# uber-research/UPSNet

Hardware: NVIDIA H100
Metric: panoptic images/sec at 1024x2048 (higher is better)
Workload: dtype bf16x3

## Files before the change

upsnet_b200/csrc/dcn_win.cu:

```cuda
#include <cuda.h>
#include <cuda_bf16.h>

#include "common.cuh"
#include "tc_ptx.cuh"
#include "tc_params.cuh"

namespace ups {

constexpr int DW_BM = 128;
constexpr int DW_WW = 32, DW_WH = 20;
constexpr int DW_PLANE = DW_WW * DW_WH * 32;
constexpr int DW_WIN_BYTES = 2 * DW_PLANE;
constexpr int DW_WIN_BUFS = 2;
constexpr int DW_KHW = 9;
constexpr int DW_GROUPS = 2;
constexpr int DW_EPI_PITCH = 36;
constexpr uint32_t DW_EPI_BYTES = DW_BM * DW_EPI_PITCH * 4;

constexpr uint32_t DW_OFF_BARS = 0;
constexpr uint32_t DW_OFF_STATS = 192;
constexpr uint32_t DW_OFF_ORG = 256;
constexpr uint32_t DW_OFF_TW = 512;
constexpr uint32_t DW_OFF_TP = DW_OFF_TW + DW_KHW * DW_BM * 16;
constexpr uint32_t DW_OFF_STAGES = DW_OFF_TP + DW_KHW * DW_BM * 4;
static_assert(DW_OFF_STAGES % 1024 == 0, "stage buffers need 1024-byte alignment (SWIZZLE_128B)");

template <int BN> struct DwCfg {
  static constexpr int NCW = BN == 128 ? 2 : 1;
  static constexpr int FRAGS = 2 / NCW;
  static constexpr int BK = BN == 128 ? 32 : 64;
  static constexpr int SPK = BK / 16;
  static constexpr int ROWB = BK * 2;
  static constexpr int CONSUMERS = 128 * NCW;
  static constexpr int WARP_TMAB = CONSUMERS / 32, WARP_TMAW = WARP_TMAB + 1, WARP_PROD0 = WARP_TMAB + 4;
  static constexpr int GROUP = 4 * (SPK / 2) * 32;
  static constexpr int PRODUCERS = GROUP * DW_GROUPS;
  static constexpr int THREADS = WARP_PROD0 * 32 + PRODUCERS;
  static constexpr int WARPGROUPS = THREADS / 128;
  static constexpr int REGS_LAUNCH = 16384 / (32 * ((THREADS / 32 + 3) / 4)) / 8 * 8;
  static constexpr int REGS_TMA = 32, REGS_CONSUMER = 128;
  static_assert(NCW * REGS_CONSUMER + REGS_TMA + (PRODUCERS / 128) * REGS_LAUNCH <= WARPGROUPS * REGS_LAUNCH,
                "setmaxnreg budgets exceed the CTA's register allocation");
  static constexpr int TABLE_IT = (DW_KHW * DW_BM + PRODUCERS - 1) / PRODUCERS;
  static constexpr uint32_t A_BYTES = 2 * DW_BM * ROWB;
  static constexpr uint32_t B_BYTES = BN * ROWB;
  static constexpr uint32_t STAGE_BYTES = 2 * B_BYTES + A_BYTES;
  static_assert(STAGE_BYTES % 1024 == 0, "stages must keep the 1024-byte alignment of the swizzled tiles");
  static constexpr int STAGES = BN == 128 ? 3 : 2;
  static_assert(STAGES <= 3, "the barrier map holds three stages");
  static constexpr uint32_t OFF_WIN = DW_OFF_STAGES + STAGES * STAGE_BYTES;
  static constexpr uint32_t OFF_EPI = OFF_WIN + DW_WIN_BUFS * DW_WIN_BYTES;
  static constexpr uint32_t SMEM = OFF_EPI + DW_EPI_BYTES + 1024;
  static_assert(SMEM <= 227 * 1024, "shared memory exceeds 227 KB");
};
template <int ROWB> __device__ __forceinline__ uint32_t dw_chunk(uint32_t j, uint32_t r) {
  return ROWB == 128 ? (j ^ (r & 7u)) : (j ^ ((r >> 1) & 3u));
}

struct DwParams {
  const void* x;
  const float* offset;
  const float* mask;
  const float* bias;
  void* y;
  int N, H, W, Cin, Cout, Cout_pad, Ho, Wo, ph, pw, dh, dw, relu, BN, tile_w, tile_h;
};

template <int BN>
__global__ void __launch_bounds__(DwCfg<BN>::THREADS, 1)
dcn_win_kernel(const __grid_constant__ CUtensorMap tm_x, const __grid_constant__ CUtensorMap tm_w, const __grid_constant__ DwParams p) {
  using C = DwCfg<BN>;
  constexpr int DW_PRODUCERS = C::PRODUCERS, DW_CONSUMERS = C::CONSUMERS;
  constexpr int DW_WARP_TMAB = C::WARP_TMAB, DW_WARP_TMAW = C::WARP_TMAW, DW_WARP_PROD0 = C::WARP_PROD0;
  constexpr int DW_BK = C::BK, SPK = C::SPK, ROWB = C::ROWB;
  extern __shared__ __align__(1024) uint8_t smem_dyn[];
  const uint32_t raw = smem_u32(smem_dyn);
  const uint32_t base = (raw + 1023u) & ~1023u;
  uint8_t* sm = smem_dyn + (base - raw);

  const int tid = threadIdx.x, warp = tid >> 5, lane = tid & 31;
  const uint32_t b_bytes = C::B_BYTES;
  const uint32_t stage_bytes = C::STAGE_BYTES;
  constexpr uint32_t NST = C::STAGES, NWB = DW_WIN_BUFS;
  const uint32_t win_base = base + C::OFF_WIN;
  float* stf = reinterpret_cast<float*>(sm + C::OFF_EPI);
  const uint32_t bar_fa = base + DW_OFF_BARS;
  const uint32_t bar_fb = bar_fa + 24;
  const uint32_t bar_em = bar_fa + 48;
  const uint32_t bar_wf = bar_fa + 104;
  const uint32_t bar_we = bar_fa + 120;
  const uint32_t bar_og = bar_fa + 136;
  int* stats = reinterpret_cast<int*>(sm + DW_OFF_STATS);
  int4* org = reinterpret_cast<int4*>(sm + DW_OFF_ORG);
  float4* tw = reinterpret_cast<float4*>(sm + DW_OFF_TW);
  int* tp = reinterpret_cast<int*>(sm + DW_OFF_TP);

  const int HoWo = p.Ho * p.Wo;
  const int nsc = p.Cin / 16;
  const int num_kb = nsc * DW_KHW / SPK;
  const int n_tiles = p.Cout_pad / BN;
  const int TW = p.tile_w, TH = p.tile_h;
  const int tw_shift = TW == 16 ? 4 : 3;
  const int tiles_w = (p.Wo + TW - 1) / TW, tiles_h = (p.Ho + TH - 1) / TH;
  const long long num_tiles = (long long)p.N * tiles_w * tiles_h * n_tiles;

  if (warp == 0) {
    if (lane == 0) {
      for (int s = 0; s < C::STAGES; ++s) {
        mbar_init(bar_fa + 8 * s, C::GROUP / 32);
        mbar_init(bar_fb + 8 * s, 1);
        mbar_init(bar_em + 8 * s, DW_CONSUMERS / 32);
      }
      for (int s = 0; s < 2; ++s) {
        mbar_init(bar_wf + 8 * s, 1);
        mbar_init(bar_we + 8 * s, DW_PRODUCERS / 32);
        mbar_init(bar_og + 8 * s, 1);
      }
      fence_mbar_init();
      for (int i = 0; i < 2; ++i) {
        stats[i * 8 + 0] = 0x7fffffff; stats[i * 8 + 1] = 0x7fffffff;
        stats[i * 8 + 2] = -0x7fffffff; stats[i * 8 + 3] = -0x7fffffff;
        stats[i * 8 + 4] = 0; stats[i * 8 + 5] = 0; stats[i * 8 + 6] = 0; stats[i * 8 + 7] = 0;
      }
    }
    __syncwarp();
  }
  if (warp == DW_WARP_TMAB && lane == 0) prefetch_tmap(&tm_w);
  if (warp == DW_WARP_TMAW && lane == 0) prefetch_tmap(&tm_x);
  __syncthreads();

  if (warp >= DW_WARP_PROD0) {
    const int pt = tid - DW_WARP_PROD0 * 32;
    const int pw = warp - DW_WARP_PROD0;
    const int group = pw / (C::GROUP / 32);
    const int u = (pw >> 2) & (SPK / 2 - 1);
    const int quad = pw & 3;
    const int r = quad * 32 + lane;
    const __nv_bfloat16* xh = reinterpret_cast<const __nv_bfloat16*>(p.x);
    uint32_t g0 = 0, wf0 = 0;
    uint32_t wf_ready = 0;
    uint32_t tile_it = 0;
    for (long long tile = blockIdx.x; tile < num_tiles; tile += gridDim.x, ++tile_it) {
      const long long mt = tile / n_tiles;
      const int tx = (int)(mt % tiles_w), ty = (int)((mt / tiles_w) % tiles_h), n = (int)(mt / ((long long)tiles_w * tiles_h));
      const int par = (int)(tile_it & 1u);
      constexpr int TIT = C::TABLE_IT;
      float4 ewv[TIT];
      int ehl[TIT], ewl[TIT];
      bool evalid[TIT];
      int mnw = 0x7fffffff, mnh = 0x7fffffff, mxw = -0x7fffffff, mxh = -0x7fffffff, sw_ = 0, sh_ = 0, cnt = 0;
#pragma unroll
      for (int it = 0; it < TIT; ++it) {
        const int e = pt + it * DW_PRODUCERS;
        ewv[it] = make_float4(0.f, 0.f, 0.f, 0.f);
        ehl[it] = 0; ewl[it] = 0; evalid[it] = false;
        if (e < DW_KHW * DW_BM) {
          const int tap = e >> 7, rr = e & 127;
          const int ry = rr >> tw_shift;
          const int wo = tx * TW + (rr & (TW - 1)), ho = ty * TH + ry;
          if (ry < TH && wo < p.Wo && ho < p.Ho) {
            const int pp = ho * p.Wo + wo;
            const int ki = tap / 3, kj = tap - ki * 3;
            const float* offp = p.offset + ((size_t)n * 2 * DW_KHW + 2 * tap) * HoWo + pp;
            const float oh = __ldg(offp), ow = __ldg(offp + HoWo);
            const float h = (float)(ho - p.ph + ki * p.dh) + oh;
            const float w = (float)(wo - p.pw + kj * p.dw) + ow;
            if (h > -1.f && w > -1.f && h < (float)p.H && w < (float)p.W) {
              const int hl = (int)floorf(h), wl = (int)floorf(w), hh = hl + 1, wh = wl + 1;
              const float lh = h - hl, lw = w - wl, ch = 1.f - lh, cw = 1.f - lw;
              const bool t_ok = hl >= 0, b_ok = hh <= p.H - 1, l_ok = wl >= 0, r_ok = wh <= p.W - 1;
              float m = 1.f;
              if (p.mask) m = __ldg(p.mask + ((size_t)n * DW_KHW + tap) * HoWo + pp);
              ewv[it].x = (t_ok && l_ok) ? ch * cw * m : 0.f;
              ewv[it].y = (t_ok && r_ok) ? ch * lw * m : 0.f;
              ewv[it].z = (b_ok && l_ok) ? lh * cw * m : 0.f;
              ewv[it].w = (b_ok && r_ok) ? lh * lw * m : 0.f;
              ehl[it] = hl; ewl[it] = wl; evalid[it] = true;
              mnw = min(mnw, wl); mxw = max(mxw, wl + 1); mnh = min(mnh, hl); mxh = max(mxh, hl + 1);
              sw_ += wl; sh_ += hl; ++cnt;
            }
          }
        }
      }
      mnw = __reduce_min_sync(0xffffffffu, mnw); mnh = __reduce_min_sync(0xffffffffu, mnh);
      mxw = __reduce_max_sync(0xffffffffu, mxw); mxh = __reduce_max_sync(0xffffffffu, mxh);
      sw_ = __reduce_add_sync(0xffffffffu, sw_); sh_ = __reduce_add_sync(0xffffffffu, sh_);
      cnt = __reduce_add_sync(0xffffffffu, cnt);
      if (lane == 0 && cnt > 0) {
        int* st = stats + par * 8;
        atomicMin(st + 0, mnw); atomicMin(st + 1, mnh); atomicMax(st + 2, mxw); atomicMax(st + 3, mxh);
        atomicAdd(st + 4, sw_); atomicAdd(st + 5, sh_); atomicAdd(st + 6, cnt);
      }
      named_bar<1, DW_PRODUCERS>();
      int ox = 0, oy = 0;
      {
        const int* st = stats + par * 8;
        const int c = st[6];
        if (c > 0) {
          const int a = st[0], b = st[1], cc = st[2], d = st[3];
          ox = (cc - a + 1 <= DW_WW) ? a : (int)floorf((float)st[4] / (float)c + 1.0f) - DW_WW / 2;
          oy = (d - b + 1 <= DW_WH) ? b : (int)floorf((float)st[5] / (float)c + 1.0f) - DW_WH / 2;
        }
      }
#pragma unroll
      for (int it = 0; it < TIT; ++it) {
        const int e = pt + it * DW_PRODUCERS;
        if (e < DW_KHW * DW_BM) {
          int code = 0;
          if (evalid[it]) {
            const int dx = ewl[it] - ox, dy = ehl[it] - oy;
            if (dx >= 0 && dx + 1 < DW_WW && dy >= 0 && dy + 1 < DW_WH) code = (dy * DW_WW + dx) * 32;
            else code = (int)(0x80000000u | ((uint32_t)(ehl[it] + 1) << 15) | (uint32_t)(ewl[it] + 1));
          }
          tw[e] = ewv[it];
          tp[e] = code;
        }
      }
      if (pt == 0) {
        org[par] = make_int4(ox, oy, n, 0);
        int* so = stats + (par ^ 1) * 8;
        so[0] = 0x7fffffff; so[1] = 0x7fffffff; so[2] = -0x7fffffff; so[3] = -0x7fffffff; so[4] = 0; so[5] = 0; so[6] = 0;
        mbar_arrive(bar_og + 8 * par);
      }
      named_bar<1, DW_PRODUCERS>();
      const __nv_bfloat16* ximg = xh + (size_t)n * p.H * p.W * (size_t)(2 * p.Cin);

      int rel = 0;
      for (int kb = (int)((uint32_t)(group - (int)g0) & 1u); kb < num_kb; kb += DW_GROUPS) {
        const uint32_t g = g0 + (uint32_t)kb;
        const uint32_t s = g % NST, it = g / NST;
        mbar_wait(bar_em + 8 * s, (it & 1u) ^ 1u);
        const uint32_t a_row = base + DW_OFF_STAGES + s * stage_bytes + 2 * b_bytes + (uint32_t)r * (uint32_t)ROWB;
#pragma unroll 1
        for (int pass = 0; pass < 4; ++pass) {
          const int sl = 2 * u + (pass >> 1), half = pass & 1;
          const int q = kb * SPK + sl;
          const int sc = q / DW_KHW, tap = q - sc * DW_KHW;
          const uint32_t wf = wf0 + (uint32_t)sc;
          if (wf >= wf_ready) {
            mbar_wait(bar_wf + 8 * (wf % NWB), (wf / NWB) & 1u);
            wf_ready = wf + 1;
          }
          const uint32_t wbuf = win_base + (wf % NWB) * (uint32_t)DW_WIN_BYTES;
          const int code = tp[tap * DW_BM + r];
          const uint32_t a_off = dw_chunk<ROWB>((uint32_t)(sl * 2 + half), (uint32_t)r) << 4;
          const float4 wv = tw[tap * DW_BM + r];
          uint4 hc[4], lc[4];
          if (code >= 0) {
            const uint32_t cl = (uint32_t)code, cr = cl + 32u;
            const uint32_t al = wbuf + cl + ((((cl >> 7) & 1u) ^ (uint32_t)half) << 4);
            const uint32_t ar = wbuf + cr + ((((cr >> 7) & 1u) ^ (uint32_t)half) << 4);
            hc[0] = lds128(al); hc[1] = lds128(ar); hc[2] = lds128(al + DW_WW * 32); hc[3] = lds128(ar + DW_WW * 32);
            lc[0] = lds128(al + DW_PLANE); lc[1] = lds128(ar + DW_PLANE);
            lc[2] = lds128(al + DW_PLANE + DW_WW * 32); lc[3] = lds128(ar + DW_PLANE + DW_WW * 32);
          } else {
            const int hl = (int)(((uint32_t)code >> 15) & 0xffffu) - 1, wl = (int)((uint32_t)code & 0x7fffu) - 1;
            const int h0 = max(hl, 0), h1 = min(hl + 1, p.H - 1), w0 = max(wl, 0), w1 = min(wl + 1, p.W - 1);
            const size_t pc = (size_t)(2 * p.Cin);
            const int cg = sc * 16 + half * 8;
            const __nv_bfloat16* b00 = ximg + ((size_t)h0 * p.W + w0) * pc + cg;
            const __nv_bfloat16* b01 = ximg + ((size_t)h0 * p.W + w1) * pc + cg;
            const __nv_bfloat16* b10 = ximg + ((size_t)h1 * p.W + w0) * pc + cg;
            const __nv_bfloat16* b11 = ximg + ((size_t)h1 * p.W + w1) * pc + cg;
            hc[0] = __ldg(reinterpret_cast<const uint4*>(b00)); lc[0] = __ldg(reinterpret_cast<const uint4*>(b00 + p.Cin));
            hc[1] = __ldg(reinterpret_cast<const uint4*>(b01)); lc[1] = __ldg(reinterpret_cast<const uint4*>(b01 + p.Cin));
            hc[2] = __ldg(reinterpret_cast<const uint4*>(b10)); lc[2] = __ldg(reinterpret_cast<const uint4*>(b10 + p.Cin));
            hc[3] = __ldg(reinterpret_cast<const uint4*>(b11)); lc[3] = __ldg(reinterpret_cast<const uint4*>(b11 + p.Cin));
          }
          const float wf4[4] = {wv.x, wv.y, wv.z, wv.w};
          unsigned long long acc[4] = {0ull, 0ull, 0ull, 0ull};
          __nv_bfloat162 lacc[4];
#pragma unroll
          for (int i = 0; i < 4; ++i) {
            const uint32_t hw_[4] = {hc[i].x, hc[i].y, hc[i].z, hc[i].w};
            const uint32_t lw_[4] = {lc[i].x, lc[i].y, lc[i].z, lc[i].w};
            const __nv_bfloat162 wb = __float2bfloat162_rn(wf4[i]);
            unsigned long long wp;
            asm("mov.b64 %0, {%1, %1};" : "=l"(wp) : "r"(__float_as_uint(wf4[i])));
#pragma unroll
            for (int qq = 0; qq < 4; ++qq) {
              unsigned long long hp;
              asm("mov.b64 %0, {%1, %2};" : "=l"(hp) : "r"(hw_[qq] << 16), "r"(hw_[qq] & 0xffff0000u));
              acc[qq] = f32x2_fma(wp, hp, acc[qq]);
              const __nv_bfloat162 lv = *reinterpret_cast<const __nv_bfloat162*>(&lw_[qq]);
              lacc[qq] = i == 0 ? __hmul2(wb, lv) : __hfma2(wb, lv, lacc[qq]);
            }
          }
          uint32_t ohi[4], olo[4];
#pragma unroll
          for (int qq = 0; qq < 4; ++qq) {
            const uint32_t lw = *reinterpret_cast<const uint32_t*>(&lacc[qq]);
            unsigned long long lp;
            asm("mov.b64 %0, {%1, %2};" : "=l"(lp) : "r"(lw << 16), "r"(lw & 0xffff0000u));
            acc[qq] = f32x2_add(acc[qq], lp);
            uint32_t a0, a1;
            asm("mov.b64 {%0, %1}, %2;" : "=r"(a0), "=r"(a1) : "l"(acc[qq]));
            const float v0 = __uint_as_float(a0), v1 = __uint_as_float(a1);
            ohi[qq] = pack_bf16x2(v0, v1);
            olo[qq] = pack_bf16x2(v0 - __uint_as_float(ohi[qq] << 16), v1 - __uint_as_float(ohi[qq] & 0xffff0000u));
          }
          sts128(a_row + a_off, make_uint4(ohi[0], ohi[1], ohi[2], ohi[3]));
          sts128(a_row + DW_BM * ROWB + a_off, make_uint4(olo[0], olo[1], olo[2], olo[3]));
        }
        fence_proxy_async();
        __syncwarp();
        if (lane == 0) {
          mbar_arrive(bar_fa + 8 * s);
          while (rel < nsc && DW_KHW * (rel + 1) <= SPK * (kb + DW_GROUPS)) {
            mbar_arrive(bar_we + 8 * ((wf0 + (uint32_t)rel) % NWB));
            ++rel;
          }
        }
        rel = __shfl_sync(0xffffffffu, rel, 0);
      }
      if (lane == 0) {
        while (rel < nsc) { mbar_arrive(bar_we + 8 * ((wf0 + (uint32_t)rel) % NWB)); ++rel; }
      }
      __syncwarp();
      g0 += (uint32_t)num_kb;
      wf0 += (uint32_t)nsc;
    }
  } else if (warp >= DW_WARP_TMAB) {
    setmaxnreg_dec<C::REGS_TMA>();
    if (warp == DW_WARP_TMAW && lane == 0) {
      uint32_t wf = 0, ti = 0;
      for (long long tile = blockIdx.x; tile < num_tiles; tile += gridDim.x, ++ti) {
        const uint32_t par = ti & 1u;
        mbar_wait(bar_og + 8 * par, (ti >> 1) & 1u);
        const volatile int* ov = reinterpret_cast<const volatile int*>(&org[par]);
        const int4 o = make_int4(ov[0], ov[1], ov[2], 0);
        for (int f = 0; f < nsc; ++f, ++wf) {
          const uint32_t b = wf % NWB;
          mbar_wait(bar_we + 8 * b, ((wf / NWB) & 1u) ^ 1u);
          mbar_arrive_expect_tx(bar_wf + 8 * b, (uint32_t)DW_WIN_BYTES);
          const uint32_t dst = win_base + b * (uint32_t)DW_WIN_BYTES;
          tma_load_4d(dst, &tm_x, bar_wf + 8 * b, f * 16, o.x, o.y, o.z);
          tma_load_4d(dst + (uint32_t)DW_PLANE, &tm_x, bar_wf + 8 * b, p.Cin + f * 16, o.x, o.y, o.z);
        }
      }
    } else if (warp == DW_WARP_TMAB && lane == 0) {
      uint32_t g = 0;
      for (long long tile = blockIdx.x; tile < num_tiles; tile += gridDim.x) {
        const int n0 = (int)(tile % n_tiles) * BN;
        for (int kb = 0; kb < num_kb; ++kb, ++g) {
          const uint32_t s = g % NST, it = g / NST;
          mbar_wait(bar_em + 8 * s, (it & 1u) ^ 1u);
          const uint32_t stage = base + DW_OFF_STAGES + s * stage_bytes;
          mbar_arrive_expect_tx(bar_fb + 8 * s, 2 * b_bytes);
          tma_load_2d(stage, &tm_w, bar_fb + 8 * s, kb * DW_BK, n0);
          tma_load_2d(stage + b_bytes, &tm_w, bar_fb + 8 * s, kb * DW_BK, p.Cout_pad + n0);
        }
      }
    }
    __syncwarp();
  } else {
    setmaxnreg_inc<C::REGS_CONSUMER>();
    constexpr int FRAGS = C::FRAGS;
    const int wg = warp >> 2;
    const uint32_t dhi = ROWB == 128 ? wg_desc_hi(8 * ROWB) : wg_desc_hi_sw64(8 * ROWB);
    float d[FRAGS][BN / 2];
    constexpr uint32_t h16 = 64u * ROWB / 16u;
    __nv_bfloat16* yb = reinterpret_cast<__nv_bfloat16*>(p.y);
    uint32_t s = 0, ph = 0;
    for (long long tile = blockIdx.x; tile < num_tiles; tile += gridDim.x) {
      const long long mt = tile / n_tiles;
      const int n0 = (int)(tile % n_tiles) * BN;
      const int tx = (int)(mt % tiles_w), ty = (int)((mt / tiles_w) % tiles_h), n = (int)(mt / ((long long)tiles_w * tiles_h));
      int prev = -1;
      for (int kb = 0; kb < num_kb; ++kb) {
        mbar_wait(bar_fb + 8 * s, ph);
        mbar_wait(bar_fa + 8 * s, ph);
        const uint32_t st0 = base + DW_OFF_STAGES + s * stage_bytes;
        const uint32_t b_hi = wg_desc_lo(st0), b_lo = wg_desc_lo(st0 + b_bytes);
        const uint32_t a_hi = wg_desc_lo(st0 + 2 * b_bytes) + (uint32_t)(wg * FRAGS) * h16;
        const uint32_t a_lo = wg_desc_lo(st0 + 2 * b_bytes + DW_BM * ROWB) + (uint32_t)(wg * FRAGS) * h16;
        wgmma_fence();
#pragma unroll
        for (uint32_t k = 0; k < SPK; ++k) {
          const uint32_t acc = (kb | k) ? 1u : 0u;
          const uint64_t bh = wg_desc(b_hi + 2 * k, dhi), bl = wg_desc(b_lo + 2 * k, dhi);
#pragma unroll
          for (int f = 0; f < FRAGS; ++f) Wgmma<BN>::mma(d[f], wg_desc(a_lo + f * h16 + 2 * k, dhi), bh, acc);
#pragma unroll
          for (int f = 0; f < FRAGS; ++f) Wgmma<BN>::mma(d[f], wg_desc(a_hi + f * h16 + 2 * k, dhi), bl, 1u);
#pragma unroll
          for (int f = 0; f < FRAGS; ++f) Wgmma<BN>::mma(d[f], wg_desc(a_hi + f * h16 + 2 * k, dhi), bh, 1u);
        }
        wgmma_commit();
        wgmma_wait<1>();
#pragma unroll
        for (int f = 0; f < FRAGS; ++f) wgmma_fence_acc(d[f]);
        if (prev >= 0 && lane == 0) mbar_arrive(bar_em + 8 * prev);
        prev = (int)s;
        if (++s == NST) { s = 0; ph ^= 1u; }
      }
      wgmma_wait<0>();
#pragma unroll
      for (int f = 0; f < FRAGS; ++f) wgmma_fence_acc(d[f]);
      if (prev >= 0 && lane == 0) mbar_arrive(bar_em + 8 * prev);

      const int t = tid & 127;
      const int m = FRAGS == 2 ? t : 64 * wg + (t & 63);
      const int csub = FRAGS == 2 ? 0 : 16 * (t >> 6), cstep = FRAGS == 2 ? 16 : 32;
      const int ry = m >> tw_shift;
      const int wo = tx * TW + (m & (TW - 1)), ho = ty * TH + ry;
      const bool row_ok = ry < TH && wo < p.Wo && ho < p.Ho;
      __nv_bfloat16* yp = yb + (((size_t)n * p.Ho + ho) * p.Wo + wo) * (size_t)(2 * p.Cout);
      const uint32_t trow = smem_u32(stf + (size_t)m * DW_EPI_PITCH);
      for (int c32 = 0; c32 < BN; c32 += 32) {
        if (n0 + c32 >= p.Cout) break;
        named_bar(2 + wg, 128);
#pragma unroll
        for (int c = 0; c < BN; c += 32)
          if (c == c32) {
#pragma unroll
            for (int f = 0; f < FRAGS; ++f) acc_stage<BN, 32>(d[f], stf, DW_EPI_PITCH, 64 * (wg * FRAGS + f), c);
          }
        named_bar(2 + wg, 128);
        for (int cb = c32 + csub; cb < c32 + 32 && cb < BN; cb += cstep) {
          if (n0 + cb >= p.Cout) break;
          uint32_t rr[16];
          acc_ld16(trow + (uint32_t)(cb - c32) * 4u, rr);
          if (!row_ok) continue;
          const int co = n0 + cb;
          float o[16];
#pragma unroll
          for (int e = 0; e < 16; ++e) o[e] = __uint_as_float(rr[e]);
          if (p.bias) {
            if (co + 16 <= p.Cout) {
#pragma unroll
              for (int e4 = 0; e4 < 4; ++e4) {
                const float4 bv = __ldg(reinterpret_cast<const float4*>(p.bias + co) + e4);
                o[4 * e4] += bv.x; o[4 * e4 + 1] += bv.y; o[4 * e4 + 2] += bv.z; o[4 * e4 + 3] += bv.w;
              }
            } else {
#pragma unroll
              for (int e = 0; e < 16; ++e)
                if (co + e < p.Cout) o[e] += __ldg(p.bias + co + e);
            }
          }
          if (p.relu) {
#pragma unroll
            for (int e = 0; e < 16; ++e) o[e] = fmaxf(o[e], 0.f);
          }
          uint32_t hw[8], lw[8];
#pragma unroll
          for (int e = 0; e < 8; ++e) {
            hw[e] = pack_bf16x2(o[2 * e], o[2 * e + 1]);
            lw[e] = pack_bf16x2(o[2 * e] - __uint_as_float(hw[e] << 16), o[2 * e + 1] - __uint_as_float(hw[e] & 0xffff0000u));
          }
          uint4* dh_ = reinterpret_cast<uint4*>(yp + co);
          uint4* dl_ = reinterpret_cast<uint4*>(yp + p.Cout + co);
          dh_[0] = make_uint4(hw[0], hw[1], hw[2], hw[3]); dh_[1] = make_uint4(hw[4], hw[5], hw[6], hw[7]);
          dl_[0] = make_uint4(lw[0], lw[1], lw[2], lw[3]); dl_[1] = make_uint4(lw[4], lw[5], lw[6], lw[7]);
        }
      }
    }
  }
}

__global__ void dcn_win_pack_kernel(const float* __restrict__ w, int Cout, int Cin, int Cout_pad, int K,
                                    uint16_t* __restrict__ hi, uint16_t* __restrict__ lo) {
  const size_t total = (size_t)Cout_pad * K;
  for (size_t i = (size_t)blockIdx.x * blockDim.x + threadIdx.x; i < total; i += (size_t)gridDim.x * blockDim.x) {
    const int kk = (int)(i % (size_t)K), co = (int)(i / (size_t)K);
    const int sc = kk / (16 * DW_KHW), rem = kk - sc * 16 * DW_KHW, tap = rem >> 4, c = sc * 16 + (rem & 15);
    const float v = co < Cout ? w[((size_t)co * Cin + c) * DW_KHW + tap] : 0.f;
    const __nv_bfloat16 h = __float2bfloat16_rn(v);
    const __nv_bfloat16 l = __float2bfloat16_rn(v - __bfloat162float(h));
    hi[i] = *reinterpret_cast<const uint16_t*>(&h);
    lo[i] = *reinterpret_cast<const uint16_t*>(&l);
  }
}

static bool dw_supported(int Cin, int Cout, int kh, int kw) {
  return kh == 3 && kw == 3 && Cin % 64 == 0 && Cin >= 64 && Cout >= 1;
}

}

extern "C" int upsnet_dcn_packed_weight_bytes(int Cout, int Cin, int kh, int kw, size_t* bytes) {
  if (!bytes || Cout <= 0 || Cin <= 0) return UPSNET_E_BADARG;
  if (!ups::dw_supported(Cin, Cout, kh, kw)) return UPSNET_E_UNSUPPORTED;
  *bytes = (size_t)2 * ups::cout_pad(Cout) * (size_t)(9 * Cin) * sizeof(uint16_t);
  return 0;
}

extern "C" int upsnet_dcn_pack_weight(const float* weight, int Cout, int Cin, int kh, int kw, void* packed, void* stream) {
  if (!weight || !packed || Cout <= 0 || Cin <= 0) return UPSNET_E_BADARG;
  if (!ups::dw_supported(Cin, Cout, kh, kw)) return UPSNET_E_UNSUPPORTED;
  const int Cout_pad = ups::cout_pad(Cout), K = 9 * Cin;
  uint16_t* hi = reinterpret_cast<uint16_t*>(packed);
  uint16_t* lo = hi + (size_t)Cout_pad * K;
  const size_t total = (size_t)Cout_pad * K;
  int blocks = (int)((total + 255) / 256);
  if (blocks > ups::kNumSMs * 16) blocks = ups::kNumSMs * 16;
  ups::dcn_win_pack_kernel<<<blocks, 256, 0, (cudaStream_t)stream>>>(weight, Cout, Cin, Cout_pad, K, hi, lo);
  UPS_CHECK_LAUNCH();
  return 0;
}

static int g_dw_force_bn = 0;

extern "C" int upsnet_dcn_set_tile_n(int bn) {
  if (bn != 0 && bn != 32 && bn != 128) return UPSNET_E_BADARG;
  g_dw_force_bn = bn;
  return 0;
}

extern "C" int upsnet_dcn_pair_forward(const void* x_pair, const float* offset, const float* mask, const void* packed,
                                       const float* bias, void* y_pair, int N, int H, int W, int Cin, int Cout, int kh,
                                       int kw, int pad_h, int pad_w, int dil_h, int dil_w, int epi_flags, void* stream) {
  using namespace ups;
  if (!x_pair || !offset || !packed || !y_pair) return UPSNET_E_BADARG;
  if (N <= 0 || H <= 0 || W <= 0 || Cin <= 0 || Cout <= 0 || pad_h < 0 || pad_w < 0 || dil_h <= 0 || dil_w <= 0) return UPSNET_E_BADARG;
  if (!dw_supported(Cin, Cout, kh, kw)) return UPSNET_E_UNSUPPORTED;
  if ((Cout % 16) != 0) return UPSNET_E_UNSUPPORTED;
  if (H >= 32767 || W >= 32767) return UPSNET_E_UNSUPPORTED;
  if ((((uintptr_t)x_pair) & 15) || (((uintptr_t)packed) & 15) || (((uintptr_t)y_pair) & 15) || (bias && (((uintptr_t)bias) & 15)))
    return UPSNET_E_UNSUPPORTED;
  DwParams p{};
  p.x = x_pair; p.offset = offset; p.mask = mask; p.bias = bias; p.y = y_pair;
  p.N = N; p.H = H; p.W = W; p.Cin = Cin; p.Cout = Cout; p.Cout_pad = cout_pad(Cout);
  p.ph = pad_h; p.pw = pad_w; p.dh = dil_h; p.dw = dil_w;
  p.Ho = conv_out_size(H, pad_h, dil_h, 3, 1);
  p.Wo = conv_out_size(W, pad_w, dil_w, 3, 1);
  if (p.Ho <= 0 || p.Wo <= 0) return UPSNET_E_BADARG;
  p.relu = (epi_flags & UPSNET_EPI_RELU) ? 1 : 0;
  const int sms = num_sms();
  p.tile_w = 16; p.tile_h = 8;
  auto dtiles = [&]() { return (long long)p.N * ((p.Wo + p.tile_w - 1) / p.tile_w) * ((p.Ho + p.tile_h - 1) / p.tile_h) * (p.Cout_pad / p.BN); };
  p.BN = 128;
  const bool wide_ok = p.Cout_pad % 128 == 0;
  const bool wide = wide_ok && (g_dw_force_bn == 128 || (g_dw_force_bn == 0 && dtiles() >= sms / 4));
  if (!wide) p.BN = 32;
  if (!wide && dtiles() < sms / 2) { p.tile_w = 8; p.tile_h = 8; }
  if (!wide && dtiles() < sms / 2) { p.tile_h = 4; }
  const long long num_tiles = dtiles();
  if (num_tiles <= 0) return 0;
  const int bk = wide ? DwCfg<128>::BK : DwCfg<32>::BK;
  const size_t smem = wide ? DwCfg<128>::SMEM : DwCfg<32>::SMEM;
  EncodeTiledFn enc = tma_encoder();
  if (!enc) return UPSNET_E_UNSUPPORTED;
  CUtensorMap tm_x, tm_w;
  {
    const cuuint64_t dx[4] = {(cuuint64_t)(2 * Cin), (cuuint64_t)W, (cuuint64_t)H, (cuuint64_t)N};
    const cuuint64_t sx[3] = {(cuuint64_t)(2 * Cin) * 2, (cuuint64_t)W * (2 * Cin) * 2, (cuuint64_t)H * W * (2 * Cin) * 2};
    const cuuint32_t bx[4] = {16, DW_WW, DW_WH, 1};
    const cuuint32_t es[4] = {1, 1, 1, 1};
    if (enc(&tm_x, CU_TENSOR_MAP_DATA_TYPE_BFLOAT16, 4, const_cast<void*>(x_pair), dx, sx, bx, es, CU_TENSOR_MAP_INTERLEAVE_NONE,
            CU_TENSOR_MAP_SWIZZLE_32B, CU_TENSOR_MAP_L2_PROMOTION_L2_128B, CU_TENSOR_MAP_FLOAT_OOB_FILL_NONE) != CUDA_SUCCESS)
      return UPSNET_E_UNSUPPORTED;
    const cuuint64_t dwt[2] = {(cuuint64_t)(9 * Cin), (cuuint64_t)(2 * p.Cout_pad)};
    const cuuint64_t sw[1] = {(cuuint64_t)(9 * Cin) * 2};
    const cuuint32_t bw[2] = {(cuuint32_t)bk, (cuuint32_t)p.BN};
    if (enc(&tm_w, CU_TENSOR_MAP_DATA_TYPE_BFLOAT16, 2, const_cast<void*>(packed), dwt, sw, bw, es, CU_TENSOR_MAP_INTERLEAVE_NONE,
            bk == 64 ? CU_TENSOR_MAP_SWIZZLE_128B : CU_TENSOR_MAP_SWIZZLE_64B, CU_TENSOR_MAP_L2_PROMOTION_L2_256B,
            CU_TENSOR_MAP_FLOAT_OOB_FILL_NONE) != CUDA_SUCCESS)
      return UPSNET_E_UNSUPPORTED;
  }
  static PerDeviceOnce configured;
  if (configured.need()) {
    UPS_CUDA(cudaFuncSetAttribute(dcn_win_kernel<32>, cudaFuncAttributeMaxDynamicSharedMemorySize, 227 * 1024));
    UPS_CUDA(cudaFuncSetAttribute(dcn_win_kernel<128>, cudaFuncAttributeMaxDynamicSharedMemorySize, 227 * 1024));
  }
  dim3 grid((unsigned)(num_tiles < sms ? num_tiles : sms));
  if (wide)
    dcn_win_kernel<128><<<grid, DwCfg<128>::THREADS, smem, (cudaStream_t)stream>>>(tm_x, tm_w, p);
  else
    dcn_win_kernel<32><<<grid, DwCfg<32>::THREADS, smem, (cudaStream_t)stream>>>(tm_x, tm_w, p);
  UPS_CHECK_LAUNCH();
  return 0;
}
```

upsnet_b200/csrc/tc_ptx.cuh:

```cuda
#pragma once
#include <cuda.h>
#include <cuda_bf16.h>
#include <cstdint>
#include <cstdio>

namespace ups {

__device__ __forceinline__ uint32_t smem_u32(const void* p) { return (uint32_t)__cvta_generic_to_shared(p); }

__device__ __forceinline__ void mbar_init(uint32_t bar, uint32_t count) {
  asm volatile("mbarrier.init.shared::cta.b64 [%0], %1;" ::"r"(bar), "r"(count));
}
__device__ __forceinline__ void mbar_arrive(uint32_t bar) {
  asm volatile("mbarrier.arrive.shared::cta.b64 _, [%0];" ::"r"(bar) : "memory");
}
__device__ __forceinline__ bool mbar_try_wait(uint32_t bar, uint32_t parity) {
  uint32_t ok;
  asm volatile(
      "{\n\t.reg .pred p;\n\t"
      "mbarrier.try_wait.parity.shared::cta.b64 p, [%1], %2;\n\t"
      "selp.u32 %0, 1, 0, p;\n\t}"
      : "=r"(ok) : "r"(bar), "r"(parity) : "memory");
  return ok != 0;
}
__device__ __forceinline__ void mbar_wait(uint32_t bar, uint32_t parity) {
  uint32_t spins = 0;
  long long t0 = 0;
  while (!mbar_try_wait(bar, parity)) {
    if ((++spins & 1023u) == 0) {
      const long long now = clock64();
      if (t0 == 0) t0 = now;
      else if (now - t0 > 4000000000LL) __trap();
    }
  }
}
__device__ __forceinline__ void fence_mbar_init() { asm volatile("fence.mbarrier_init.release.cluster;" ::: "memory"); }
__device__ __forceinline__ void fence_proxy_async() { asm volatile("fence.proxy.async.shared::cta;" ::: "memory"); }

__device__ __forceinline__ void mbar_arrive_expect_tx(uint32_t bar, uint32_t bytes) {
  asm volatile("mbarrier.arrive.expect_tx.shared::cta.b64 _, [%0], %1;" ::"r"(bar), "r"(bytes) : "memory");
}
__device__ __forceinline__ void tma_load_2d(uint32_t dst, const CUtensorMap* tm, uint32_t bar, int c0, int c1) {
  asm volatile(
      "cp.async.bulk.tensor.2d.shared::cluster.global.tile.mbarrier::complete_tx::bytes [%0], [%1, {%3, %4}], [%2];"
      ::"r"(dst), "l"(reinterpret_cast<uint64_t>(tm)), "r"(bar), "r"(c0), "r"(c1) : "memory");
}
__device__ __forceinline__ void tma_load_4d(uint32_t dst, const CUtensorMap* tm, uint32_t bar, int c0, int c1, int c2, int c3) {
  asm volatile(
      "cp.async.bulk.tensor.4d.shared::cluster.global.tile.mbarrier::complete_tx::bytes [%0], [%1, {%3, %4, %5, %6}], [%2];"
      ::"r"(dst), "l"(reinterpret_cast<uint64_t>(tm)), "r"(bar), "r"(c0), "r"(c1), "r"(c2), "r"(c3) : "memory");
}
__device__ __forceinline__ void tma_load_5d(uint32_t dst, const CUtensorMap* tm, uint32_t bar, int c0, int c1, int c2, int c3, int c4) {
  asm volatile(
      "cp.async.bulk.tensor.5d.shared::cluster.global.tile.mbarrier::complete_tx::bytes [%0], [%1, {%3, %4, %5, %6, %7}], [%2];"
      ::"r"(dst), "l"(reinterpret_cast<uint64_t>(tm)), "r"(bar), "r"(c0), "r"(c1), "r"(c2), "r"(c3), "r"(c4) : "memory");
}
__device__ __forceinline__ void tma_store_4d(const CUtensorMap* tm, uint32_t src, int c0, int c1, int c2, int c3) {
  asm volatile(
      "cp.async.bulk.tensor.4d.global.shared::cta.tile.bulk_group [%0, {%2, %3, %4, %5}], [%1];"
      ::"l"(reinterpret_cast<uint64_t>(tm)), "r"(src), "r"(c0), "r"(c1), "r"(c2), "r"(c3) : "memory");
}
__device__ __forceinline__ void bulk_commit() { asm volatile("cp.async.bulk.commit_group;" ::: "memory"); }
__device__ __forceinline__ void bulk_wait_read0() { asm volatile("cp.async.bulk.wait_group.read 0;" ::: "memory"); }
__device__ __forceinline__ void bulk_wait_read1() { asm volatile("cp.async.bulk.wait_group.read 1;" ::: "memory"); }
__device__ __forceinline__ void bulk_wait0() { asm volatile("cp.async.bulk.wait_group 0;" ::: "memory"); }
__device__ __forceinline__ void prefetch_tmap(const CUtensorMap* tm) {
  asm volatile("prefetch.tensormap [%0];" ::"l"(reinterpret_cast<uint64_t>(tm)) : "memory");
}

template <int R> __device__ __forceinline__ void setmaxnreg_inc() { asm volatile("setmaxnreg.inc.sync.aligned.u32 %0;" ::"n"(R)); }
template <int R> __device__ __forceinline__ void setmaxnreg_dec() { asm volatile("setmaxnreg.dec.sync.aligned.u32 %0;" ::"n"(R)); }

template <int N> struct Wgmma;
template <> struct Wgmma<32> {
  static __device__ __forceinline__ void mma(float (&d)[16], uint64_t da, uint64_t db, uint32_t accumulate) {
    asm volatile(
        "{\n\t.reg .pred p;\n\tsetp.ne.b32 p, %18, 0;\n\t"
        "wgmma.mma_async.sync.aligned.m64n32k16.f32.bf16.bf16 {%0, %1, %2, %3, %4, %5, %6, %7, %8, %9, %10, %11, %12, %13, %14, %15}, %16, %17, p, 1, 1, 0, 0;\n\t}"
        : "+f"(d[0]), "+f"(d[1]), "+f"(d[2]), "+f"(d[3]), "+f"(d[4]), "+f"(d[5]), "+f"(d[6]), "+f"(d[7]), "+f"(d[8]), "+f"(d[9]), "+f"(d[10]), "+f"(d[11]), "+f"(d[12]), "+f"(d[13]), "+f"(d[14]), "+f"(d[15])
        : "l"(da), "l"(db), "r"(accumulate));
  }
};
template <> struct Wgmma<64> {
  static __device__ __forceinline__ void mma(float (&d)[32], uint64_t da, uint64_t db, uint32_t accumulate) {
    asm volatile(
        "{\n\t.reg .pred p;\n\tsetp.ne.b32 p, %34, 0;\n\t"
        "wgmma.mma_async.sync.aligned.m64n64k16.f32.bf16.bf16 {%0, %1, %2, %3, %4, %5, %6, %7, %8, %9, %10, %11, %12, %13, %14, %15, %16, %17, %18, %19, %20, %21, %22, %23, %24, %25, %26, %27, %28, %29, %30, %31}, %32, %33, p, 1, 1, 0, 0;\n\t}"
        : "+f"(d[0]), "+f"(d[1]), "+f"(d[2]), "+f"(d[3]), "+f"(d[4]), "+f"(d[5]), "+f"(d[6]), "+f"(d[7]), "+f"(d[8]), "+f"(d[9]), "+f"(d[10]), "+f"(d[11]), "+f"(d[12]), "+f"(d[13]), "+f"(d[14]), "+f"(d[15]), "+f"(d[16]), "+f"(d[17]), "+f"(d[18]), "+f"(d[19]), "+f"(d[20]), "+f"(d[21]), "+f"(d[22]), "+f"(d[23]), "+f"(d[24]), "+f"(d[25]), "+f"(d[26]), "+f"(d[27]), "+f"(d[28]), "+f"(d[29]), "+f"(d[30]), "+f"(d[31])
        : "l"(da), "l"(db), "r"(accumulate));
  }
};
template <> struct Wgmma<96> {
  static __device__ __forceinline__ void mma(float (&d)[48], uint64_t da, uint64_t db, uint32_t accumulate) {
    asm volatile(
        "{\n\t.reg .pred p;\n\tsetp.ne.b32 p, %50, 0;\n\t"
        "wgmma.mma_async.sync.aligned.m64n96k16.f32.bf16.bf16 {%0, %1, %2, %3, %4, %5, %6, %7, %8, %9, %10, %11, %12, %13, %14, %15, %16, %17, %18, %19, %20, %21, %22, %23, %24, %25, %26, %27, %28, %29, %30, %31, %32, %33, %34, %35, %36, %37, %38, %39, %40, %41, %42, %43, %44, %45, %46, %47}, %48, %49, p, 1, 1, 0, 0;\n\t}"
        : "+f"(d[0]), "+f"(d[1]), "+f"(d[2]), "+f"(d[3]), "+f"(d[4]), "+f"(d[5]), "+f"(d[6]), "+f"(d[7]), "+f"(d[8]), "+f"(d[9]), "+f"(d[10]), "+f"(d[11]), "+f"(d[12]), "+f"(d[13]), "+f"(d[14]), "+f"(d[15]), "+f"(d[16]), "+f"(d[17]), "+f"(d[18]), "+f"(d[19]), "+f"(d[20]), "+f"(d[21]), "+f"(d[22]), "+f"(d[23]), "+f"(d[24]), "+f"(d[25]), "+f"(d[26]), "+f"(d[27]), "+f"(d[28]), "+f"(d[29]), "+f"(d[30]), "+f"(d[31]), "+f"(d[32]), "+f"(d[33]), "+f"(d[34]), "+f"(d[35]), "+f"(d[36]), "+f"(d[37]), "+f"(d[38]), "+f"(d[39]), "+f"(d[40]), "+f"(d[41]), "+f"(d[42]), "+f"(d[43]), "+f"(d[44]), "+f"(d[45]), "+f"(d[46]), "+f"(d[47])
        : "l"(da), "l"(db), "r"(accumulate));
  }
};
template <> struct Wgmma<128> {
  static __device__ __forceinline__ void mma(float (&d)[64], uint64_t da, uint64_t db, uint32_t accumulate) {
    asm volatile(
        "{\n\t.reg .pred p;\n\tsetp.ne.b32 p, %66, 0;\n\t"
        "wgmma.mma_async.sync.aligned.m64n128k16.f32.bf16.bf16 {%0, %1, %2, %3, %4, %5, %6, %7, %8, %9, %10, %11, %12, %13, %14, %15, %16, %17, %18, %19, %20, %21, %22, %23, %24, %25, %26, %27, %28, %29, %30, %31, %32, %33, %34, %35, %36, %37, %38, %39, %40, %41, %42, %43, %44, %45, %46, %47, %48, %49, %50, %51, %52, %53, %54, %55, %56, %57, %58, %59, %60, %61, %62, %63}, %64, %65, p, 1, 1, 0, 0;\n\t}"
        : "+f"(d[0]), "+f"(d[1]), "+f"(d[2]), "+f"(d[3]), "+f"(d[4]), "+f"(d[5]), "+f"(d[6]), "+f"(d[7]), "+f"(d[8]), "+f"(d[9]), "+f"(d[10]), "+f"(d[11]), "+f"(d[12]), "+f"(d[13]), "+f"(d[14]), "+f"(d[15]), "+f"(d[16]), "+f"(d[17]), "+f"(d[18]), "+f"(d[19]), "+f"(d[20]), "+f"(d[21]), "+f"(d[22]), "+f"(d[23]), "+f"(d[24]), "+f"(d[25]), "+f"(d[26]), "+f"(d[27]), "+f"(d[28]), "+f"(d[29]), "+f"(d[30]), "+f"(d[31]), "+f"(d[32]), "+f"(d[33]), "+f"(d[34]), "+f"(d[35]), "+f"(d[36]), "+f"(d[37]), "+f"(d[38]), "+f"(d[39]), "+f"(d[40]), "+f"(d[41]), "+f"(d[42]), "+f"(d[43]), "+f"(d[44]), "+f"(d[45]), "+f"(d[46]), "+f"(d[47]), "+f"(d[48]), "+f"(d[49]), "+f"(d[50]), "+f"(d[51]), "+f"(d[52]), "+f"(d[53]), "+f"(d[54]), "+f"(d[55]), "+f"(d[56]), "+f"(d[57]), "+f"(d[58]), "+f"(d[59]), "+f"(d[60]), "+f"(d[61]), "+f"(d[62]), "+f"(d[63])
        : "l"(da), "l"(db), "r"(accumulate));
  }
};
template <> struct Wgmma<256> {
  static __device__ __forceinline__ void mma(float (&d)[128], uint64_t da, uint64_t db, uint32_t accumulate) {
    asm volatile(
        "{\n\t.reg .pred p;\n\tsetp.ne.b32 p, %130, 0;\n\t"
        "wgmma.mma_async.sync.aligned.m64n256k16.f32.bf16.bf16 {%0, %1, %2, %3, %4, %5, %6, %7, %8, %9, %10, %11, %12, %13, %14, %15, %16, %17, %18, %19, %20, %21, %22, %23, %24, %25, %26, %27, %28, %29, %30, %31, %32, %33, %34, %35, %36, %37, %38, %39, %40, %41, %42, %43, %44, %45, %46, %47, %48, %49, %50, %51, %52, %53, %54, %55, %56, %57, %58, %59, %60, %61, %62, %63, %64, %65, %66, %67, %68, %69, %70, %71, %72, %73, %74, %75, %76, %77, %78, %79, %80, %81, %82, %83, %84, %85, %86, %87, %88, %89, %90, %91, %92, %93, %94, %95, %96, %97, %98, %99, %100, %101, %102, %103, %104, %105, %106, %107, %108, %109, %110, %111, %112, %113, %114, %115, %116, %117, %118, %119, %120, %121, %122, %123, %124, %125, %126, %127}, %128, %129, p, 1, 1, 0, 0;\n\t}"
        : "+f"(d[0]), "+f"(d[1]), "+f"(d[2]), "+f"(d[3]), "+f"(d[4]), "+f"(d[5]), "+f"(d[6]), "+f"(d[7]), "+f"(d[8]), "+f"(d[9]), "+f"(d[10]), "+f"(d[11]), "+f"(d[12]), "+f"(d[13]), "+f"(d[14]), "+f"(d[15]), "+f"(d[16]), "+f"(d[17]), "+f"(d[18]), "+f"(d[19]), "+f"(d[20]), "+f"(d[21]), "+f"(d[22]), "+f"(d[23]), "+f"(d[24]), "+f"(d[25]), "+f"(d[26]), "+f"(d[27]), "+f"(d[28]), "+f"(d[29]), "+f"(d[30]), "+f"(d[31]), "+f"(d[32]), "+f"(d[33]), "+f"(d[34]), "+f"(d[35]), "+f"(d[36]), "+f"(d[37]), "+f"(d[38]), "+f"(d[39]), "+f"(d[40]), "+f"(d[41]), "+f"(d[42]), "+f"(d[43]), "+f"(d[44]), "+f"(d[45]), "+f"(d[46]), "+f"(d[47]), "+f"(d[48]), "+f"(d[49]), "+f"(d[50]), "+f"(d[51]), "+f"(d[52]), "+f"(d[53]), "+f"(d[54]), "+f"(d[55]), "+f"(d[56]), "+f"(d[57]), "+f"(d[58]), "+f"(d[59]), "+f"(d[60]), "+f"(d[61]), "+f"(d[62]), "+f"(d[63]), "+f"(d[64]), "+f"(d[65]), "+f"(d[66]), "+f"(d[67]), "+f"(d[68]), "+f"(d[69]), "+f"(d[70]), "+f"(d[71]), "+f"(d[72]), "+f"(d[73]), "+f"(d[74]), "+f"(d[75]), "+f"(d[76]), "+f"(d[77]), "+f"(d[78]), "+f"(d[79]), "+f"(d[80]), "+f"(d[81]), "+f"(d[82]), "+f"(d[83]), "+f"(d[84]), "+f"(d[85]), "+f"(d[86]), "+f"(d[87]), "+f"(d[88]), "+f"(d[89]), "+f"(d[90]), "+f"(d[91]), "+f"(d[92]), "+f"(d[93]), "+f"(d[94]), "+f"(d[95]), "+f"(d[96]), "+f"(d[97]), "+f"(d[98]), "+f"(d[99]), "+f"(d[100]), "+f"(d[101]), "+f"(d[102]), "+f"(d[103]), "+f"(d[104]), "+f"(d[105]), "+f"(d[106]), "+f"(d[107]), "+f"(d[108]), "+f"(d[109]), "+f"(d[110]), "+f"(d[111]), "+f"(d[112]), "+f"(d[113]), "+f"(d[114]), "+f"(d[115]), "+f"(d[116]), "+f"(d[117]), "+f"(d[118]), "+f"(d[119]), "+f"(d[120]), "+f"(d[121]), "+f"(d[122]), "+f"(d[123]), "+f"(d[124]), "+f"(d[125]), "+f"(d[126]), "+f"(d[127])
        : "l"(da), "l"(db), "r"(accumulate));
  }
};

__device__ __forceinline__ void wgmma_fence() { asm volatile("wgmma.fence.sync.aligned;" ::: "memory"); }
__device__ __forceinline__ void wgmma_commit() { asm volatile("wgmma.commit_group.sync.aligned;" ::: "memory"); }
template <int PENDING> __device__ __forceinline__ void wgmma_wait() {
  asm volatile("wgmma.wait_group.sync.aligned %0;" ::"n"(PENDING) : "memory");
}
template <int R> __device__ __forceinline__ void wgmma_fence_acc(float (&d)[R]) {
#pragma unroll
  for (int i = 0; i < R; ++i) asm volatile("" : "+f"(d[i])::"memory");
}

__device__ __forceinline__ uint32_t wg_desc_lo(uint32_t smem_addr) { return ((smem_addr >> 4) & 0x3fffu) | (1u << 16); }
__device__ __forceinline__ uint32_t wg_desc_hi(uint32_t sbo_bytes) { return (sbo_bytes >> 4) | (1u << 30); }
__device__ __forceinline__ uint32_t wg_desc_hi_sw64(uint32_t sbo_bytes) { return (sbo_bytes >> 4) | (2u << 30); }
__device__ __forceinline__ uint64_t wg_desc(uint32_t lo, uint32_t hi) { return ((uint64_t)hi << 32) | lo; }

template <int N, int NC>
__device__ __forceinline__ void acc_stage(const float (&d)[N / 2], float* buf, int pitch, int row0, int c0) {
  const int t = threadIdx.x & 127, l = t & 31;
  const int r = row0 + 16 * (t >> 5) + (l >> 2);
#pragma unroll
  for (int i = 0; i < N / 8; ++i) {
    if (8 * i < c0 || 8 * i >= c0 + NC) continue;
    const int c = 8 * i - c0 + 2 * (l & 3);
    *reinterpret_cast<float2*>(buf + (size_t)r * pitch + c) = make_float2(d[4 * i], d[4 * i + 1]);
    *reinterpret_cast<float2*>(buf + (size_t)(r + 8) * pitch + c) = make_float2(d[4 * i + 2], d[4 * i + 3]);
  }
}
__device__ __forceinline__ void acc_ld16(uint32_t addr, uint32_t (&r)[16]) {
#pragma unroll
  for (int i = 0; i < 4; ++i)
    asm volatile("ld.shared.v4.b32 {%0, %1, %2, %3}, [%4];"
                 : "=r"(r[4 * i]), "=r"(r[4 * i + 1]), "=r"(r[4 * i + 2]), "=r"(r[4 * i + 3]) : "r"(addr + 16u * i));
}
__device__ __forceinline__ uint4 lds128(uint32_t addr) {
  uint4 v;
  asm volatile("ld.shared.v4.u32 {%0, %1, %2, %3}, [%4];" : "=r"(v.x), "=r"(v.y), "=r"(v.z), "=r"(v.w) : "r"(addr));
  return v;
}
__device__ __forceinline__ void sts128(uint32_t addr, const uint4& v) {
  asm volatile("st.shared.v4.u32 [%0], {%1, %2, %3, %4};" ::"r"(addr), "r"(v.x), "r"(v.y), "r"(v.z), "r"(v.w) : "memory");
}
__device__ __forceinline__ uint32_t lds32(uint32_t addr) {
  uint32_t v;
  asm volatile("ld.shared.b32 %0, [%1];" : "=r"(v) : "r"(addr));
  return v;
}
__device__ __forceinline__ void sts32(uint32_t addr, uint32_t v) {
  asm volatile("st.shared.b32 [%0], %1;" ::"r"(addr), "r"(v) : "memory");
}
__device__ __forceinline__ void named_bar(int id, int count) { asm volatile("bar.sync %0, %1;" ::"r"(id), "r"(count) : "memory"); }
template <int ID, int COUNT> __device__ __forceinline__ void named_bar() { asm volatile("bar.sync %0, %1;" ::"n"(ID), "n"(COUNT) : "memory"); }

__device__ __forceinline__ void cp_async16(uint32_t dst_smem, const void* src) {
  asm volatile("cp.async.cg.shared.global [%0], [%1], 16;" ::"r"(dst_smem), "l"(src) : "memory");
}
__device__ __forceinline__ void cp_async16_zfill(uint32_t dst_smem, const void* src, uint32_t src_bytes) {
  asm volatile("cp.async.cg.shared.global [%0], [%1], 16, %2;" ::"r"(dst_smem), "l"(src), "r"(src_bytes) : "memory");
}
__device__ __forceinline__ void cp_async_commit() { asm volatile("cp.async.commit_group;" ::: "memory"); }
__device__ __forceinline__ void cp_async_wait_all() { asm volatile("cp.async.wait_group 0;" ::: "memory"); }
__device__ __forceinline__ void cp_async_wait_but2() { asm volatile("cp.async.wait_group 2;" ::: "memory"); }

__device__ __forceinline__ uint32_t pack_bf16x2(float a, float b) {
  __nv_bfloat162 v = __floats2bfloat162_rn(a, b);
  return *reinterpret_cast<uint32_t*>(&v);
}
__device__ __forceinline__ void ldg256(const void* p, uint4& lo, uint4& hi) {
  lo = __ldg(reinterpret_cast<const uint4*>(p));
  hi = __ldg(reinterpret_cast<const uint4*>(p) + 1);
}
__device__ __forceinline__ unsigned long long f32x2_fma(unsigned long long a, unsigned long long b, unsigned long long c) {
  const float r0 = fmaf(__uint_as_float((uint32_t)a), __uint_as_float((uint32_t)b), __uint_as_float((uint32_t)c));
  const float r1 = fmaf(__uint_as_float((uint32_t)(a >> 32)), __uint_as_float((uint32_t)(b >> 32)), __uint_as_float((uint32_t)(c >> 32)));
  return ((unsigned long long)__float_as_uint(r1) << 32) | __float_as_uint(r0);
}
__device__ __forceinline__ unsigned long long f32x2_add(unsigned long long a, unsigned long long b) {
  const float r0 = __uint_as_float((uint32_t)a) + __uint_as_float((uint32_t)b);
  const float r1 = __uint_as_float((uint32_t)(a >> 32)) + __uint_as_float((uint32_t)(b >> 32));
  return ((unsigned long long)__float_as_uint(r1) << 32) | __float_as_uint(r0);
}
__device__ __forceinline__ uint32_t bf2_blend(const uint4& w, uint32_t a, uint32_t b, uint32_t d, uint32_t e) {
  const __nv_bfloat162 wa = *reinterpret_cast<const __nv_bfloat162*>(&w.x), wb = *reinterpret_cast<const __nv_bfloat162*>(&w.y);
  const __nv_bfloat162 wd = *reinterpret_cast<const __nv_bfloat162*>(&w.z), we = *reinterpret_cast<const __nv_bfloat162*>(&w.w);
  __nv_bfloat162 acc = __hmul2(wa, *reinterpret_cast<const __nv_bfloat162*>(&a));
  acc = __hfma2(wb, *reinterpret_cast<const __nv_bfloat162*>(&b), acc);
  acc = __hfma2(wd, *reinterpret_cast<const __nv_bfloat162*>(&d), acc);
  acc = __hfma2(we, *reinterpret_cast<const __nv_bfloat162*>(&e), acc);
  return *reinterpret_cast<const uint32_t*>(&acc);
}
__device__ __forceinline__ float bf16_round(float a) { return __bfloat162float(__float2bfloat16_rn(a)); }

}
```

Before: 93.04.

## Fuse deformable sampling into consumer warps and feed A from registers via wgmma RS

Removes the separate producer warp groups that bilinearly sampled the deformable-conv input into swizzled shared-memory A tiles. The 256 consumer threads now compute the sampled fragments themselves and pass them straight to register-sourced wgmma (m64nNk16 RS variants). Only the weight B tiles stay in staged shared memory, which frees space to deepen the pipeline to 6 or 8 stages. In exchange, the consumer warps carry both the gather math and the MMA on a register budget that setmaxnreg now recomputes, and sampling latency is no longer hidden by separate warps.

New measurement: 92.72 (median of 6 runs). Within noise of the previous version (-0.3%).

```diff
diff --git a/upsnet_b200/csrc/dcn_win.cu b/upsnet_b200/csrc/dcn_win.cu
--- a/upsnet_b200/csrc/dcn_win.cu
+++ b/upsnet_b200/csrc/dcn_win.cu
@@ -13,9 +13,9 @@
 constexpr int DW_WIN_BYTES = 2 * DW_PLANE;
 constexpr int DW_WIN_BUFS = 2;
 constexpr int DW_KHW = 9;
-constexpr int DW_GROUPS = 2;
 constexpr int DW_EPI_PITCH = 36;
 constexpr uint32_t DW_EPI_BYTES = DW_BM * DW_EPI_PITCH * 4;
+constexpr int DW_MAX_STAGES = 8;
 
 constexpr uint32_t DW_OFF_BARS = 0;
 constexpr uint32_t DW_OFF_STATS = 192;
@@ -26,36 +26,28 @@
 static_assert(DW_OFF_STAGES % 1024 == 0, "stage buffers need 1024-byte alignment (SWIZZLE_128B)");
 
 template <int BN> struct DwCfg {
-  static constexpr int NCW = BN == 128 ? 2 : 1;
-  static constexpr int FRAGS = 2 / NCW;
   static constexpr int BK = BN == 128 ? 32 : 64;
   static constexpr int SPK = BK / 16;
   static constexpr int ROWB = BK * 2;
-  static constexpr int CONSUMERS = 128 * NCW;
-  static constexpr int WARP_TMAB = CONSUMERS / 32, WARP_TMAW = WARP_TMAB + 1, WARP_PROD0 = WARP_TMAB + 4;
-  static constexpr int GROUP = 4 * (SPK / 2) * 32;
-  static constexpr int PRODUCERS = GROUP * DW_GROUPS;
-  static constexpr int THREADS = WARP_PROD0 * 32 + PRODUCERS;
+  static constexpr int CONSUMERS = 256;
+  static constexpr int WARP_TMAB = CONSUMERS / 32, WARP_TMAW = WARP_TMAB + 1;
+  static constexpr int THREADS = CONSUMERS + 128;
   static constexpr int WARPGROUPS = THREADS / 128;
   static constexpr int REGS_LAUNCH = 16384 / (32 * ((THREADS / 32 + 3) / 4)) / 8 * 8;
-  static constexpr int REGS_TMA = 32, REGS_CONSUMER = 128;
-  static_assert(NCW * REGS_CONSUMER + REGS_TMA + (PRODUCERS / 128) * REGS_LAUNCH <= WARPGROUPS * REGS_LAUNCH,
-                "setmaxnreg budgets exceed the CTA's register allocation");
-  static constexpr int TABLE_IT = (DW_KHW * DW_BM + PRODUCERS - 1) / PRODUCERS;
-  static constexpr uint32_t A_BYTES = 2 * DW_BM * ROWB;
+  static constexpr int REGS_TMA = 32;
+  static constexpr int REGS_CONSUMER = (WARPGROUPS * REGS_LAUNCH - REGS_TMA) / 2 / 8 * 8;
+  static_assert(2 * REGS_CONSUMER + REGS_TMA <= WARPGROUPS * REGS_LAUNCH, "setmaxnreg budgets exceed the CTA's register allocation");
+  static constexpr int TABLE_IT = (DW_KHW * DW_BM + CONSUMERS - 1) / CONSUMERS;
   static constexpr uint32_t B_BYTES = BN * ROWB;
-  static constexpr uint32_t STAGE_BYTES = 2 * B_BYTES + A_BYTES;
+  static constexpr uint32_t STAGE_BYTES = 2 * B_BYTES;
   static_assert(STAGE_BYTES % 1024 == 0, "stages must keep the 1024-byte alignment of the swizzled tiles");
-  static constexpr int STAGES = BN == 128 ? 3 : 2;
-  static_assert(STAGES <= 3, "the barrier map holds three stages");
+  static constexpr int STAGES = BN == 128 ? 6 : 8;
+  static_assert(STAGES <= DW_MAX_STAGES, "the barrier map holds eight stages");
   static constexpr uint32_t OFF_WIN = DW_OFF_STAGES + STAGES * STAGE_BYTES;
   static constexpr uint32_t OFF_EPI = OFF_WIN + DW_WIN_BUFS * DW_WIN_BYTES;
   static constexpr uint32_t SMEM = OFF_EPI + DW_EPI_BYTES + 1024;
   static_assert(SMEM <= 227 * 1024, "shared memory exceeds 227 KB");
 };
-template <int ROWB> __device__ __forceinline__ uint32_t dw_chunk(uint32_t j, uint32_t r) {
-  return ROWB == 128 ? (j ^ (r & 7u)) : (j ^ ((r >> 1) & 3u));
-}
 
 struct DwParams {
   const void* x;
@@ -66,12 +58,14 @@
   int N, H, W, Cin, Cout, Cout_pad, Ho, Wo, ph, pw, dh, dw, relu, BN, tile_w, tile_h;
 };
 
+struct DwFrag { uint32_t hi[4], lo[4]; };
+struct DwCorners { uint32_t hc[4][4], lc[4][4]; float4 wv[2]; };
+
 template <int BN>
 __global__ void __launch_bounds__(DwCfg<BN>::THREADS, 1)
 dcn_win_kernel(const __grid_constant__ CUtensorMap tm_x, const __grid_constant__ CUtensorMap tm_w, const __grid_constant__ DwParams p) {
   using C = DwCfg<BN>;
-  constexpr int DW_PRODUCERS = C::PRODUCERS, DW_CONSUMERS = C::CONSUMERS;
-  constexpr int DW_WARP_TMAB = C::WARP_TMAB, DW_WARP_TMAW = C::WARP_TMAW, DW_WARP_PROD0 = C::WARP_PROD0;
+  constexpr int DW_CONSUMERS = C::CONSUMERS;
   constexpr int DW_BK = C::BK, SPK = C::SPK, ROWB = C::ROWB;
   extern __shared__ __align__(1024) uint8_t smem_dyn[];
   const uint32_t raw = smem_u32(smem_dyn);
@@ -84,12 +78,11 @@
   constexpr uint32_t NST = C::STAGES, NWB = DW_WIN_BUFS;
   const uint32_t win_base = base + C::OFF_WIN;
   float* stf = reinterpret_cast<float*>(sm + C::OFF_EPI);
-  const uint32_t bar_fa = base + DW_OFF_BARS;
-  const uint32_t bar_fb = bar_fa + 24;
-  const uint32_t bar_em = bar_fa + 48;
-  const uint32_t bar_wf = bar_fa + 104;
-  const uint32_t bar_we = bar_fa + 120;
-  const uint32_t bar_og = bar_fa + 136;
+  const uint32_t bar_fb = base + DW_OFF_BARS;
+  const uint32_t bar_em = bar_fb + 8 * DW_MAX_STAGES;
+  const uint32_t bar_wf = bar_fb + 16 * DW_MAX_STAGES;
+  const uint32_t bar_we = bar_wf + 16;
+  const uint32_t bar_og = bar_wf + 32;
   int* stats = reinterpret_cast<int*>(sm + DW_OFF_STATS);
   int4* org = reinterpret_cast<int4*>(sm + DW_OFF_ORG);
   float4* tw = reinterpret_cast<float4*>(sm + DW_OFF_TW);
@@ -107,13 +100,12 @@
   if (warp == 0) {
     if (lane == 0) {
       for (int s = 0; s < C::STAGES; ++s) {
-        mbar_init(bar_fa + 8 * s, C::GROUP / 32);
         mbar_init(bar_fb + 8 * s, 1);
         mbar_init(bar_em + 8 * s, DW_CONSUMERS / 32);
       }
       for (int s = 0; s < 2; ++s) {
         mbar_init(bar_wf + 8 * s, 1);
-        mbar_init(bar_we + 8 * s, DW_PRODUCERS / 32);
+        mbar_init(bar_we + 8 * s, DW_CONSUMERS / 32);
         mbar_init(bar_og + 8 * s, 1);
       }
       fence_mbar_init();
@@ -125,204 +117,13 @@
     }
     __syncwarp();
   }
-  if (warp == DW_WARP_TMAB && lane == 0) prefetch_tmap(&tm_w);
-  if (warp == DW_WARP_TMAW && lane == 0) prefetch_tmap(&tm_x);
+  if (warp == C::WARP_TMAB && lane == 0) prefetch_tmap(&tm_w);
+  if (warp == C::WARP_TMAW && lane == 0) prefetch_tmap(&tm_x);
   __syncthreads();
 
-  if (warp >= DW_WARP_PROD0) {
-    const int pt = tid - DW_WARP_PROD0 * 32;
-    const int pw = warp - DW_WARP_PROD0;
-    const int group = pw / (C::GROUP / 32);
-    const int u = (pw >> 2) & (SPK / 2 - 1);
-    const int quad = pw & 3;
-    const int r = quad * 32 + lane;
-    const __nv_bfloat16* xh = reinterpret_cast<const __nv_bfloat16*>(p.x);
-    uint32_t g0 = 0, wf0 = 0;
-    uint32_t wf_ready = 0;
-    uint32_t tile_it = 0;
-    for (long long tile = blockIdx.x; tile < num_tiles; tile += gridDim.x, ++tile_it) {
-      const long long mt = tile / n_tiles;
-      const int tx = (int)(mt % tiles_w), ty = (int)((mt / tiles_w) % tiles_h), n = (int)(mt / ((long long)tiles_w * tiles_h));
-      const int par = (int)(tile_it & 1u);
-      constexpr int TIT = C::TABLE_IT;
-      float4 ewv[TIT];
-      int ehl[TIT], ewl[TIT];
-      bool evalid[TIT];
-      int mnw = 0x7fffffff, mnh = 0x7fffffff, mxw = -0x7fffffff, mxh = -0x7fffffff, sw_ = 0, sh_ = 0, cnt = 0;
-#pragma unroll
-      for (int it = 0; it < TIT; ++it) {
-        const int e = pt + it * DW_PRODUCERS;
-        ewv[it] = make_float4(0.f, 0.f, 0.f, 0.f);
-        ehl[it] = 0; ewl[it] = 0; evalid[it] = false;
-        if (e < DW_KHW * DW_BM) {
-          const int tap = e >> 7, rr = e & 127;
-          const int ry = rr >> tw_shift;
-          const int wo = tx * TW + (rr & (TW - 1)), ho = ty * TH + ry;
-          if (ry < TH && wo < p.Wo && ho < p.Ho) {
-            const int pp = ho * p.Wo + wo;
-            const int ki = tap / 3, kj = tap - ki * 3;
-            const float* offp = p.offset + ((size_t)n * 2 * DW_KHW + 2 * tap) * HoWo + pp;
-            const float oh = __ldg(offp), ow = __ldg(offp + HoWo);
-            const float h = (float)(ho - p.ph + ki * p.dh) + oh;
-            const float w = (float)(wo - p.pw + kj * p.dw) + ow;
-            if (h > -1.f && w > -1.f && h < (float)p.H && w < (float)p.W) {
-              const int hl = (int)floorf(h), wl = (int)floorf(w), hh = hl + 1, wh = wl + 1;
-              const float lh = h - hl, lw = w - wl, ch = 1.f - lh, cw = 1.f - lw;
-              const bool t_ok = hl >= 0, b_ok = hh <= p.H - 1, l_ok = wl >= 0, r_ok = wh <= p.W - 1;
-              float m = 1.f;
-              if (p.mask) m = __ldg(p.mask + ((size_t)n * DW_KHW + tap) * HoWo + pp);
-              ewv[it].x = (t_ok && l_ok) ? ch * cw * m : 0.f;
-              ewv[it].y = (t_ok && r_ok) ? ch * lw * m : 0.f;
-              ewv[it].z = (b_ok && l_ok) ? lh * cw * m : 0.f;
-              ewv[it].w = (b_ok && r_ok) ? lh * lw * m : 0.f;
-              ehl[it] = hl; ewl[it] = wl; evalid[it] = true;
-              mnw = min(mnw, wl); mxw = max(mxw, wl + 1); mnh = min(mnh, hl); mxh = max(mxh, hl + 1);
-              sw_ += wl; sh_ += hl; ++cnt;
-            }
-          }
-        }
-      }
-      mnw = __reduce_min_sync(0xffffffffu, mnw); mnh = __reduce_min_sync(0xffffffffu, mnh);
-      mxw = __reduce_max_sync(0xffffffffu, mxw); mxh = __reduce_max_sync(0xffffffffu, mxh);
-      sw_ = __reduce_add_sync(0xffffffffu, sw_); sh_ = __reduce_add_sync(0xffffffffu, sh_);
-      cnt = __reduce_add_sync(0xffffffffu, cnt);
-      if (lane == 0 && cnt > 0) {
-        int* st = stats + par * 8;
-        atomicMin(st + 0, mnw); atomicMin(st + 1, mnh); atomicMax(st + 2, mxw); atomicMax(st + 3, mxh);
-        atomicAdd(st + 4, sw_); atomicAdd(st + 5, sh_); atomicAdd(st + 6, cnt);
-      }
-      named_bar<1, DW_PRODUCERS>();
-      int ox = 0, oy = 0;
-      {
-        const int* st = stats + par * 8;
-        const int c = st[6];
-        if (c > 0) {
-          const int a = st[0], b = st[1], cc = st[2], d = st[3];
-          ox = (cc - a + 1 <= DW_WW) ? a : (int)floorf((float)st[4] / (float)c + 1.0f) - DW_WW / 2;
-          oy = (d - b + 1 <= DW_WH) ? b : (int)floorf((float)st[5] / (float)c + 1.0f) - DW_WH / 2;
-        }
-      }
-#pragma unroll
-      for (int it = 0; it < TIT; ++it) {
-        const int e = pt + it * DW_PRODUCERS;
-        if (e < DW_KHW * DW_BM) {
-          int code = 0;
-          if (evalid[it]) {
-            const int dx = ewl[it] - ox, dy = ehl[it] - oy;
-            if (dx >= 0 && dx + 1 < DW_WW && dy >= 0 && dy + 1 < DW_WH) code = (dy * DW_WW + dx) * 32;
-            else code = (int)(0x80000000u | ((uint32_t)(ehl[it] + 1) << 15) | (uint32_t)(ewl[it] + 1));
-          }
-          tw[e] = ewv[it];
-          tp[e] = code;
-        }
-      }
-      if (pt == 0) {
-        org[par] = make_int4(ox, oy, n, 0);
-        int* so = stats + (par ^ 1) * 8;
-        so[0] = 0x7fffffff; so[1] = 0x7fffffff; so[2] = -0x7fffffff; so[3] = -0x7fffffff; so[4] = 0; so[5] = 0; so[6] = 0;
-        mbar_arrive(bar_og + 8 * par);
-      }
-      named_bar<1, DW_PRODUCERS>();
-      const __nv_bfloat16* ximg = xh + (size_t)n * p.H * p.W * (size_t)(2 * p.Cin);
-
-      int rel = 0;
-      for (int kb = (int)((uint32_t)(group - (int)g0) & 1u); kb < num_kb; kb += DW_GROUPS) {
-        const uint32_t g = g0 + (uint32_t)kb;
-        const uint32_t s = g % NST, it = g / NST;
-        mbar_wait(bar_em + 8 * s, (it & 1u) ^ 1u);
-        const uint32_t a_row = base + DW_OFF_STAGES + s * stage_bytes + 2 * b_bytes + (uint32_t)r * (uint32_t)ROWB;
-#pragma unroll 1
-        for (int pass = 0; pass < 4; ++pass) {
-          const int sl = 2 * u + (pass >> 1), half = pass & 1;
-          const int q = kb * SPK + sl;
-          const int sc = q / DW_KHW, tap = q - sc * DW_KHW;
-          const uint32_t wf = wf0 + (uint32_t)sc;
-          if (wf >= wf_ready) {
-            mbar_wait(bar_wf + 8 * (wf % NWB), (wf / NWB) & 1u);
-            wf_ready = wf + 1;
-          }
-          const uint32_t wbuf = win_base + (wf % NWB) * (uint32_t)DW_WIN_BYTES;
-          const int code = tp[tap * DW_BM + r];
-          const uint32_t a_off = dw_chunk<ROWB>((uint32_t)(sl * 2 + half), (uint32_t)r) << 4;
-          const float4 wv = tw[tap * DW_BM + r];
-          uint4 hc[4], lc[4];
-          if (code >= 0) {
-            const uint32_t cl = (uint32_t)code, cr = cl + 32u;
-            const uint32_t al = wbuf + cl + ((((cl >> 7) & 1u) ^ (uint32_t)half) << 4);
-            const uint32_t ar = wbuf + cr + ((((cr >> 7) & 1u) ^ (uint32_t)half) << 4);
-            hc[0] = lds128(al); hc[1] = lds128(ar); hc[2] = lds128(al + DW_WW * 32); hc[3] = lds128(ar + DW_WW * 32);
-            lc[0] = lds128(al + DW_PLANE); lc[1] = lds128(ar + DW_PLANE);
-            lc[2] = lds128(al + DW_PLANE + DW_WW * 32); lc[3] = lds128(ar + DW_PLANE + DW_WW * 32);
-          } else {
-            const int hl = (int)(((uint32_t)code >> 15) & 0xffffu) - 1, wl = (int)((uint32_t)code & 0x7fffu) - 1;
-            const int h0 = max(hl, 0), h1 = min(hl + 1, p.H - 1), w0 = max(wl, 0), w1 = min(wl + 1, p.W - 1);
-            const size_t pc = (size_t)(2 * p.Cin);
-            const int cg = sc * 16 + half * 8;
-            const __nv_bfloat16* b00 = ximg + ((size_t)h0 * p.W + w0) * pc + cg;
-            const __nv_bfloat16* b01 = ximg + ((size_t)h0 * p.W + w1) * pc + cg;
-            const __nv_bfloat16* b10 = ximg + ((size_t)h1 * p.W + w0) * pc + cg;
-            const __nv_bfloat16* b11 = ximg + ((size_t)h1 * p.W + w1) * pc + cg;
-            hc[0] = __ldg(reinterpret_cast<const uint4*>(b00)); lc[0] = __ldg(reinterpret_cast<const uint4*>(b00 + p.Cin));
-            hc[1] = __ldg(reinterpret_cast<const uint4*>(b01)); lc[1] = __ldg(reinterpret_cast<const uint4*>(b01 + p.Cin));
-            hc[2] = __ldg(reinterpret_cast<const uint4*>(b10)); lc[2] = __ldg(reinterpret_cast<const uint4*>(b10 + p.Cin));
-            hc[3] = __ldg(reinterpret_cast<const uint4*>(b11)); lc[3] = __ldg(reinterpret_cast<const uint4*>(b11 + p.Cin));
-          }
-          const float wf4[4] = {wv.x, wv.y, wv.z, wv.w};
-          unsigned long long acc[4] = {0ull, 0ull, 0ull, 0ull};
-          __nv_bfloat162 lacc[4];
-#pragma unroll
-          for (int i = 0; i < 4; ++i) {
-            const uint32_t hw_[4] = {hc[i].x, hc[i].y, hc[i].z, hc[i].w};
-            const uint32_t lw_[4] = {lc[i].x, lc[i].y, lc[i].z, lc[i].w};
-            const __nv_bfloat162 wb = __float2bfloat162_rn(wf4[i]);
-            unsigned long long wp;
-            asm("mov.b64 %0, {%1, %1};" : "=l"(wp) : "r"(__float_as_uint(wf4[i])));
-#pragma unroll
-            for (int qq = 0; qq < 4; ++qq) {
-              unsigned long long hp;
-              asm("mov.b64 %0, {%1, %2};" : "=l"(hp) : "r"(hw_[qq] << 16), "r"(hw_[qq] & 0xffff0000u));
-              acc[qq] = f32x2_fma(wp, hp, acc[qq]);
-              const __nv_bfloat162 lv = *reinterpret_cast<const __nv_bfloat162*>(&lw_[qq]);
-              lacc[qq] = i == 0 ? __hmul2(wb, lv) : __hfma2(wb, lv, lacc[qq]);
-            }
-          }
-          uint32_t ohi[4], olo[4];
-#pragma unroll
-          for (int qq = 0; qq < 4; ++qq) {
-            const uint32_t lw = *reinterpret_cast<const uint32_t*>(&lacc[qq]);
-            unsigned long long lp;
-            asm("mov.b64 %0, {%1, %2};" : "=l"(lp) : "r"(lw << 16), "r"(lw & 0xffff0000u));
-            acc[qq] = f32x2_add(acc[qq], lp);
-            uint32_t a0, a1;
-            asm("mov.b64 {%0, %1}, %2;" : "=r"(a0), "=r"(a1) : "l"(acc[qq]));
-            const float v0 = __uint_as_float(a0), v1 = __uint_as_float(a1);
-            ohi[qq] = pack_bf16x2(v0, v1);
-            olo[qq] = pack_bf16x2(v0 - __uint_as_float(ohi[qq] << 16), v1 - __uint_as_float(ohi[qq] & 0xffff0000u));
-          }
-          sts128(a_row + a_off, make_uint4(ohi[0], ohi[1], ohi[2], ohi[3]));
-          sts128(a_row + DW_BM * ROWB + a_off, make_uint4(olo[0], olo[1], olo[2], olo[3]));
-        }
-        fence_proxy_async();
-        __syncwarp();
-        if (lane == 0) {
-          mbar_arrive(bar_fa + 8 * s);
-          while (rel < nsc && DW_KHW * (rel + 1) <= SPK * (kb + DW_GROUPS)) {
-            mbar_arrive(bar_we + 8 * ((wf0 + (uint32_t)rel) % NWB));
-            ++rel;
-          }
-        }
-        rel = __shfl_sync(0xffffffffu, rel, 0);
-      }
-      if (lane == 0) {
-        while (rel < nsc) { mbar_arrive(bar_we + 8 * ((wf0 + (uint32_t)rel) % NWB)); ++rel; }
-      }
-      __syncwarp();
-      g0 += (uint32_t)num_kb;
-      wf0 += (uint32_t)nsc;
-    }
-  } else if (warp >= DW_WARP_TMAB) {
+  if (warp >= C::WARP_TMAB) {
     setmaxnreg_dec<C::REGS_TMA>();
-    if (warp == DW_WARP_TMAW && lane == 0) {
+    if (warp == C::WARP_TMAW && lane == 0) {
       uint32_t wf = 0, ti = 0;
       for (long long tile = blockIdx.x; tile < num_tiles; tile += gridDim.x, ++ti) {
         const uint32_t par = ti & 1u;
@@ -338,7 +139,7 @@
           tma_load_4d(dst + (uint32_t)DW_PLANE, &tm_x, bar_wf + 8 * b, p.Cin + f * 16, o.x, o.y, o.z);
         }
       }
-    } else if (warp == DW_WARP_TMAB && lane == 0) {
+    } else if (warp == C::WARP_TMAB && lane == 0) {
       uint32_t g = 0;
       for (long long tile = blockIdx.x; tile < num_tiles; tile += gridDim.x) {
         const int n0 = (int)(tile % n_tiles) * BN;
@@ -353,108 +154,290 @@
       }
     }
     __syncwarp();
-  } else {
-    setmaxnreg_inc<C::REGS_CONSUMER>();
-    constexpr int FRAGS = C::FRAGS;
-    const int wg = warp >> 2;
-    const uint32_t dhi = ROWB == 128 ? wg_desc_hi(8 * ROWB) : wg_desc_hi_sw64(8 * ROWB);
-    float d[FRAGS][BN / 2];
-    constexpr uint32_t h16 = 64u * ROWB / 16u;
-    __nv_bfloat16* yb = reinterpret_cast<__nv_bfloat16*>(p.y);
-    uint32_t s = 0, ph = 0;
-    for (long long tile = blockIdx.x; tile < num_tiles; tile += gridDim.x) {
-      const long long mt = tile / n_tiles;
-      const int n0 = (int)(tile % n_tiles) * BN;
-      const int tx = (int)(mt % tiles_w), ty = (int)((mt / tiles_w) % tiles_h), n = (int)(mt / ((long long)tiles_w * tiles_h));
-      int prev = -1;
-      for (int kb = 0; kb < num_kb; ++kb) {
-        mbar_wait(bar_fb + 8 * s, ph);
-        mbar_wait(bar_fa + 8 * s, ph);
-        const uint32_t st0 = base + DW_OFF_STAGES + s * stage_bytes;
-        const uint32_t b_hi = wg_desc_lo(st0), b_lo = wg_desc_lo(st0 + b_bytes);
-        const uint32_t a_hi = wg_desc_lo(st0 + 2 * b_bytes) + (uint32_t)(wg * FRAGS) * h16;
-        const uint32_t a_lo = wg_desc_lo(st0 + 2 * b_bytes + DW_BM * ROWB) + (uint32_t)(wg * FRAGS) * h16;
-        wgmma_fence();
-#pragma unroll
-        for (uint32_t k = 0; k < SPK; ++k) {
-          const uint32_t acc = (kb | k) ? 1u : 0u;
-          const uint64_t bh = wg_desc(b_hi + 2 * k, dhi), bl = wg_desc(b_lo + 2 * k, dhi);
-#pragma unroll
-          for (int f = 0; f < FRAGS; ++f) Wgmma<BN>::mma(d[f], wg_desc(a_lo + f * h16 + 2 * k, dhi), bh, acc);
-#pragma unroll
-          for (int f = 0; f < FRAGS; ++f) Wgmma<BN>::mma(d[f], wg_desc(a_hi + f * h16 + 2 * k, dhi), bl, 1u);
-#pragma unroll
-          for (int f = 0; f < FRAGS; ++f) Wgmma<BN>::mma(d[f], wg_desc(a_hi + f * h16 + 2 * k, dhi), bh, 1u);
+    return;
+  }
+
+  setmaxnreg_inc<C::REGS_CONSUMER>();
+  const int wg = warp >> 2;
+  const uint32_t dhi = ROWB == 128 ? wg_desc_hi(8 * ROWB) : wg_desc_hi_sw64(8 * ROWB);
+  const __nv_bfloat16* xh = reinterpret_cast<const __nv_bfloat16*>(p.x);
+  __nv_bfloat16* yb = reinterpret_cast<__nv_bfloat16*>(p.y);
+  const int r0 = 16 * warp + (lane >> 2), ra = 16 * warp + (lane & 15);
+  const int cq = 2 * (lane & 3);
+  const uint32_t a_half = (uint32_t)(lane >> 4);
+
+  constexpr int TIT = C::TABLE_IT;
+  float4 ewv[TIT];
+  int ehl[TIT], ewl[TIT];
+  bool evalid[TIT];
+  auto table_stats = [&](long long tile, int par) -> int {
+    const long long mt = tile / n_tiles;
+    const int tx = (int)(mt % tiles_w), ty = (int)((mt / tiles_w) % tiles_h), n = (int)(mt / ((long long)tiles_w * tiles_h));
+    int mnw = 0x7fffffff, mnh = 0x7fffffff, mxw = -0x7fffffff, mxh = -0x7fffffff, sw_ = 0, sh_ = 0, cnt = 0;
+#pragma unroll
+    for (int it = 0; it < TIT; ++it) {
+      const int e = tid + it * DW_CONSUMERS;
+      ewv[it] = make_float4(0.f, 0.f, 0.f, 0.f);
+      ehl[it] = 0; ewl[it] = 0; evalid[it] = false;
+      if (e < DW_KHW * DW_BM) {
+        const int tap = e >> 7, rr = e & 127;
+        const int ry = rr >> tw_shift;
+        const int wo = tx * TW + (rr & (TW - 1)), ho = ty * TH + ry;
+        if (ry < TH && wo < p.Wo && ho < p.Ho) {
+          const int pp = ho * p.Wo + wo;
+          const int ki = tap / 3, kj = tap - ki * 3;
+          const float* offp = p.offset + ((size_t)n * 2 * DW_KHW + 2 * tap) * HoWo + pp;
+          const float oh = __ldg(offp), ow = __ldg(offp + HoWo);
+          const float h = (float)(ho - p.ph + ki * p.dh) + oh;
+          const float w = (float)(wo - p.pw + kj * p.dw) + ow;
+          if (h > -1.f && w > -1.f && h < (float)p.H && w < (float)p.W) {
+            const int hl = (int)floorf(h), wl = (int)floorf(w), hh = hl + 1, wh = wl + 1;
+            const float lh = h - hl, lw = w - wl, ch = 1.f - lh, cw = 1.f - lw;
+            const bool t_ok = hl >= 0, b_ok = hh <= p.H - 1, l_ok = wl >= 0, r_ok = wh <= p.W - 1;
+            float m = 1.f;
+            if (p.mask) m = __ldg(p.mask + ((size_t)n * DW_KHW + tap) * HoWo + pp);
+            ewv[it].x = (t_ok && l_ok) ? ch * cw * m : 0.f;
+            ewv[it].y = (t_ok && r_ok) ? ch * lw * m : 0.f;
+            ewv[it].z = (b_ok && l_ok) ? lh * cw * m : 0.f;
+            ewv[it].w = (b_ok && r_ok) ? lh * lw * m : 0.f;
+            ehl[it] = hl; ewl[it] = wl; evalid[it] = true;
+            mnw = min(mnw, wl); mxw = max(mxw, wl + 1); mnh = min(mnh, hl); mxh = max(mxh, hl + 1);
+            sw_ += wl; sh_ += hl; ++cnt;
+          }
         }
-        wgmma_commit();
-        wgmma_wait<1>();
-#pragma unroll
-        for (int f = 0; f < FRAGS; ++f) wgmma_fence_acc(d[f]);
-        if (prev >= 0 && lane == 0) mbar_arrive(bar_em + 8 * prev);
-        prev = (int)s;
-        if (++s == NST) { s = 0; ph ^= 1u; }
-      }
-      wgmma_wait<0>();
-#pragma unroll
-      for (int f = 0; f < FRAGS; ++f) wgmma_fence_acc(d[f]);
-      if (prev >= 0 && lane == 0) mbar_arrive(bar_em + 8 * prev);
-
-      const int t = tid & 127;
-      const int m = FRAGS == 2 ? t : 64 * wg + (t & 63);
-      const int csub = FRAGS == 2 ? 0 : 16 * (t >> 6), cstep = FRAGS == 2 ? 16 : 32;
-      const int ry = m >> tw_shift;
-      const int wo = tx * TW + (m & (TW - 1)), ho = ty * TH + ry;
-      const bool row_ok = ry < TH && wo < p.Wo && ho < p.Ho;
-      __nv_bfloat16* yp = yb + (((size_t)n * p.Ho + ho) * p.Wo + wo) * (size_t)(2 * p.Cout);
-      const uint32_t trow = smem_u32(stf + (size_t)m * DW_EPI_PITCH);
-      for (int c32 = 0; c32 < BN; c32 += 32) {
-        if (n0 + c32 >= p.Cout) break;
-        named_bar(2 + wg, 128);
-#pragma unroll
-        for (int c = 0; c < BN; c += 32)
-          if (c == c32) {
-#pragma unroll
-            for (int f = 0; f < FRAGS; ++f) acc_stage<BN, 32>(d[f], stf, DW_EPI_PITCH, 64 * (wg * FRAGS + f), c);
+      }
+    }
+    mnw = __reduce_min_sync(0xffffffffu, mnw); mnh = __reduce_min_sync(0xffffffffu, mnh);
+    mxw = __reduce_max_sync(0xffffffffu, mxw); mxh = __reduce_max_sync(0xffffffffu, mxh);
+    sw_ = __reduce_add_sync(0xffffffffu, sw_); sh_ = __reduce_add_sync(0xffffffffu, sh_);
+    cnt = __reduce_add_sync(0xffffffffu, cnt);
+    if (lane == 0 && cnt > 0) {
+      int* st = stats + par * 8;
+      atomicMin(st + 0, mnw); atomicMin(st + 1, mnh); atomicMax(st + 2, mxw); atomicMax(st + 3, mxh);
+      atomicAdd(st + 4, sw_); atomicAdd(st + 5, sh_); atomicAdd(st + 6, cnt);
+    }
+    return n;
+  };
+  auto table_publish = [&](int par, int n) {
+    int ox = 0, oy = 0;
+    {
+      const int* st = stats + par * 8;
+      const int c = st[6];
+      if (c > 0) {
+        const int a = st[0], b = st[1], cc = st[2], d = st[3];
+        ox = (cc - a + 1 <= DW_WW) ? a : (int)floorf((float)st[4] / (float)c + 1.0f) - DW_WW / 2;
+        oy = (d - b + 1 <= DW_WH) ? b : (int)floorf((float)st[5] / (float)c + 1.0f) - DW_WH / 2;
+      }
+    }
+    if (tid == 0) {
+      org[par] = make_int4(ox, oy, n, 0);
+      int* so = stats + (par ^ 1) * 8;
+      so[0] = 0x7fffffff; so[1] = 0x7fffffff; so[2] = -0x7fffffff; so[3] = -0x7fffffff; so[4] = 0; so[5] = 0; so[6] = 0;
+      mbar_arrive(bar_og + 8 * par);
+    }
+#pragma unroll
+    for (int it = 0; it < TIT; ++it) {
+      const int e = tid + it * DW_CONSUMERS;
+      if (e < DW_KHW * DW_BM) {
+        int code = 0;
+        if (evalid[it]) {
+          const int dx = ewl[it] - ox, dy = ehl[it] - oy;
+          if (dx >= 0 && dx + 1 < DW_WW && dy >= 0 && dy + 1 < DW_WH) code = (dy * DW_WW + dx) * 32;
+          else code = (int)(0x80000000u | ((uint32_t)(ehl[it] + 1) << 15) | (uint32_t)(ewl[it] + 1));
+        }
+        tw[e] = ewv[it];
+        tp[e] = code;
+      }
+    }
+  };
+
+  uint32_t wf0 = 0;
+  const __nv_bfloat16* ximg = xh;
+  auto load = [&](int q, DwCorners& L) {
+    const int sc = q / DW_KHW, tap = q - sc * DW_KHW;
+    const uint32_t wf = wf0 + (uint32_t)sc;
+    if (tap == 0) mbar_wait(bar_wf + 8 * (wf % NWB), (wf / NWB) & 1u);
+    const uint32_t wbuf = win_base + (wf % NWB) * (uint32_t)DW_WIN_BYTES;
+    const int* tpt = tp + tap * DW_BM;
+    const float4* twt = tw + tap * DW_BM;
+    const int code_a = tpt[ra];
+    const uint32_t cl = code_a >= 0 ? (uint32_t)code_a : 0u, cr = cl + 32u;
+    const uint32_t al = wbuf + cl + ((((cl >> 7) & 1u) ^ a_half) << 4);
+    const uint32_t ar = wbuf + cr + ((((cr >> 7) & 1u) ^ a_half) << 4);
+    uint32_t (&hc)[4][4] = L.hc, (&lc)[4][4] = L.lc;
+    ldsm_x4(al, hc[0]); ldsm_x4(ar, hc[1]); ldsm_x4(al + DW_WW * 32, hc[2]); ldsm_x4(ar + DW_WW * 32, hc[3]);
+    ldsm_x4(al + DW_PLANE, lc[0]); ldsm_x4(ar + DW_PLANE, lc[1]);
+    ldsm_x4(al + DW_PLANE + DW_WW * 32, lc[2]); ldsm_x4(ar + DW_PLANE + DW_WW * 32, lc[3]);
+    L.wv[0] = twt[r0]; L.wv[1] = twt[r0 + 8];
+    const int cp[2] = {tpt[r0], tpt[r0 + 8]};
+#pragma unroll
+    for (int pi = 0; pi < 2; ++pi) {
+      if (cp[pi] < 0) {
+        const int hl = (int)(((uint32_t)cp[pi] >> 15) & 0xffffu) - 1, wl = (int)((uint32_t)cp[pi] & 0x7fffu) - 1;
+        const int h0 = max(hl, 0), h1 = min(hl + 1, p.H - 1), w0 = max(wl, 0), w1 = min(wl + 1, p.W - 1);
+        const size_t pc = (size_t)(2 * p.Cin);
+        const int cg = sc * 16 + cq;
+        const __nv_bfloat16* bc[4] = {ximg + ((size_t)h0 * p.W + w0) * pc + cg, ximg + ((size_t)h0 * p.W + w1) * pc + cg,
+                                      ximg + ((size_t)h1 * p.W + w0) * pc + cg, ximg + ((size_t)h1 * p.W + w1) * pc + cg};
+#pragma unroll
+        for (int i = 0; i < 4; ++i) {
+          hc[i][pi] = __ldg(reinterpret_cast<const uint32_t*>(bc[i]));
+          hc[i][pi + 2] = __ldg(reinterpret_cast<const uint32_t*>(bc[i] + 8));
+          lc[i][pi] = __ldg(reinterpret_cast<const uint32_t*>(bc[i] + p.Cin));
+          lc[i][pi + 2] = __ldg(reinterpret_cast<const uint32_t*>(bc[i] + p.Cin + 8));
+        }
+      }
+    }
+  };
+  auto blend = [&](int q, const DwCorners& L, DwFrag& f) {
+    const int sc = q / DW_KHW, tap = q - sc * DW_KHW;
+    const uint32_t wf = wf0 + (uint32_t)sc;
+    const uint32_t (&hc)[4][4] = L.hc, (&lc)[4][4] = L.lc;
+    const float4 (&wv)[2] = L.wv;
+#pragma unroll
+    for (int j = 0; j < 4; ++j) {
+      const float4 w4 = wv[j & 1];
+      const float wf4[4] = {w4.x, w4.y, w4.z, w4.w};
+      unsigned long long acc = 0ull;
+      __nv_bfloat162 lacc;
+#pragma unroll
+      for (int i = 0; i < 4; ++i) {
+        const __nv_bfloat162 wb = __float2bfloat162_rn(wf4[i]);
+        unsigned long long wp, hp;
+        asm("mov.b64 %0, {%1, %1};" : "=l"(wp) : "r"(__float_as_uint(wf4[i])));
+        asm("mov.b64 %0, {%1, %2};" : "=l"(hp) : "r"(hc[i][j] << 16), "r"(hc[i][j] & 0xffff0000u));
+        acc = f32x2_fma(wp, hp, acc);
+        const __nv_bfloat162 lv = *reinterpret_cast<const __nv_bfloat162*>(&lc[i][j]);
+        lacc = i == 0 ? __hmul2(wb, lv) : __hfma2(wb, lv, lacc);
+      }
+      const uint32_t lw = *reinterpret_cast<const uint32_t*>(&lacc);
+      unsigned long long lp;
+      asm("mov.b64 %0, {%1, %2};" : "=l"(lp) : "r"(lw << 16), "r"(lw & 0xffff0000u));
+      acc = f32x2_add(acc, lp);
+      uint32_t a0, a1;
+      asm("mov.b64 {%0, %1}, %2;" : "=r"(a0), "=r"(a1) : "l"(acc));
+      const float v0 = __uint_as_float(a0), v1 = __uint_as_float(a1);
+      f.hi[j] = pack_bf16x2(v0, v1);
+      f.lo[j] = pack_bf16x2(v0 - __uint_as_float(f.hi[j] << 16), v1 - __uint_as_float(f.hi[j] & 0xffff0000u));
+    }
+    if (tap == DW_KHW - 1) {
+      __syncwarp();
+      if (lane == 0) mbar_arrive(bar_we + 8 * (wf % NWB));
+    }
+  };
+
+  float d[BN / 2];
+  uint32_t s = 0, ph = 0;
+  int Q = 0;
+  auto slice = [&](int q, const DwFrag& a, DwFrag& an, const DwCorners& lcur, DwCorners& lnext) {
+    const int k = q & (SPK - 1);
+    uint32_t prev = 0;
+    if (k == 0) {
+      if (q > 0) { prev = s; if (++s == NST) { s = 0; ph ^= 1u; } }
+      mbar_wait(bar_fb + 8 * s, ph);
+    }
+    const uint32_t st0 = base + DW_OFF_STAGES + s * stage_bytes;
+    const uint64_t bh = wg_desc(wg_desc_lo(st0) + 2 * (uint32_t)k, dhi), bl = wg_desc(wg_desc_lo(st0 + b_bytes) + 2 * (uint32_t)k, dhi);
+    wgmma_fence();
+    WgmmaRS<BN>::mma(d, a.lo, bh, q > 0 ? 1u : 0u);
+    WgmmaRS<BN>::mma(d, a.hi, bl, 1u);
+    WgmmaRS<BN>::mma(d, a.hi, bh, 1u);
+    wgmma_commit();
+    wgmma_wait<1>();
+    wgmma_fence_acc(d);
+    if (k == 0 && q > 0 && lane == 0) mbar_arrive(bar_em + 8 * prev);
+    if (q + 2 < Q) load(q + 2, lnext);
+    if (q + 1 < Q) blend(q + 1, lcur, an);
+  };
+
+  long long tile = blockIdx.x;
+  uint32_t tile_it = 0;
+  {
+    const int n = table_stats(tile, 0);
+    named_bar<1, DW_CONSUMERS>();
+    table_publish(0, n);
+  }
+  for (; tile < num_tiles; tile += gridDim.x, ++tile_it) {
+    named_bar<1, DW_CONSUMERS>();
+    const long long mt = tile / n_tiles;
+    const int n0 = (int)(tile % n_tiles) * BN;
+    const int tx = (int)(mt % tiles_w), ty = (int)((mt / tiles_w) % tiles_h), n = (int)(mt / ((long long)tiles_w * tiles_h));
+    ximg = xh + (size_t)n * p.H * p.W * (size_t)(2 * p.Cin);
+    Q = nsc * DW_KHW;
+    DwFrag fa, fb;
+    DwCorners l0, l1;
+    load(0, l0);
+    load(1, l1);
+    blend(0, l0, fa);
+#pragma unroll 1
+    for (int q = 0; q < Q; q += 2) {
+      slice(q, fa, fb, l1, l0);
+      slice(q + 1, fb, fa, l0, l1);
+    }
+    wgmma_wait<0>();
+    wgmma_fence_acc(d);
+    if (lane == 0) mbar_arrive(bar_em + 8 * s);
+    if (++s == NST) { s = 0; ph ^= 1u; }
+    wf0 += (uint32_t)nsc;
+
+    const long long next = tile + gridDim.x;
+    const int par = (int)((tile_it + 1) & 1u);
+    int n_next = 0;
+    if (next < num_tiles) n_next = table_stats(next, par);
+    named_bar<1, DW_CONSUMERS>();
+    if (next < num_tiles) table_publish(par, n_next);
+
+    const int t = tid & 127;
+    const int m = 64 * wg + (t & 63);
+    const int csub = 16 * (t >> 6);
+    const int ry = m >> tw_shift;
+    const int wo = tx * TW + (m & (TW - 1)), ho = ty * TH + ry;
+    const bool row_ok = ry < TH && wo < p.Wo && ho < p.Ho;
+    __nv_bfloat16* yp = yb + (((size_t)n * p.Ho + ho) * p.Wo + wo) * (size_t)(2 * p.Cout);
+    const uint32_t trow = smem_u32(stf + (size_t)m * DW_EPI_PITCH);
+    for (int c32 = 0; c32 < BN; c32 += 32) {
+      if (n0 + c32 >= p.Cout) break;
+      named_bar(2 + wg, 128);
+#pragma unroll
+      for (int c = 0; c < BN; c += 32)
+        if (c == c32) acc_stage<BN, 32>(d, stf, DW_EPI_PITCH, 64 * wg, c);
+      named_bar(2 + wg, 128);
+      const int cb = c32 + csub;
+      if (n0 + cb >= p.Cout) continue;
+      uint32_t rr[16];
+      acc_ld16(trow + (uint32_t)csub * 4u, rr);
+      if (!row_ok) continue;
+      const int co = n0 + cb;
+      float o[16];
+#pragma unroll
+      for (int e = 0; e < 16; ++e) o[e] = __uint_as_float(rr[e]);
+      if (p.bias) {
+        if (co + 16 <= p.Cout) {
+#pragma unroll
+          for (int e4 = 0; e4 < 4; ++e4) {
+            const float4 bv = __ldg(reinterpret_cast<const float4*>(p.bias + co) + e4);
+            o[4 * e4] += bv.x; o[4 * e4 + 1] += bv.y; o[4 * e4 + 2] += bv.z; o[4 * e4 + 3] += bv.w;
           }
-        named_bar(2 + wg, 128);
-        for (int cb = c32 + csub; cb < c32 + 32 && cb < BN; cb += cstep) {
-          if (n0 + cb >= p.Cout) break;
-          uint32_t rr[16];
-          acc_ld16(trow + (uint32_t)(cb - c32) * 4u, rr);
-          if (!row_ok) continue;
-          const int co = n0 + cb;
-          float o[16];
-#pragma unroll
-          for (int e = 0; e < 16; ++e) o[e] = __uint_as_float(rr[e]);
-          if (p.bias) {
-            if (co + 16 <= p.Cout) {
-#pragma unroll
-              for (int e4 = 0; e4 < 4; ++e4) {
-                const float4 bv = __ldg(reinterpret_cast<const float4*>(p.bias + co) + e4);
-                o[4 * e4] += bv.x; o[4 * e4 + 1] += bv.y; o[4 * e4 + 2] += bv.z; o[4 * e4 + 3] += bv.w;
-              }
-            } else {
-#pragma unroll
-              for (int e = 0; e < 16; ++e)
-                if (co + e < p.Cout) o[e] += __ldg(p.bias + co + e);
-            }
-          }
-          if (p.relu) {
-#pragma unroll
-            for (int e = 0; e < 16; ++e) o[e] = fmaxf(o[e], 0.f);
-          }
-          uint32_t hw[8], lw[8];
-#pragma unroll
-          for (int e = 0; e < 8; ++e) {
-            hw[e] = pack_bf16x2(o[2 * e], o[2 * e + 1]);
-            lw[e] = pack_bf16x2(o[2 * e] - __uint_as_float(hw[e] << 16), o[2 * e + 1] - __uint_as_float(hw[e] & 0xffff0000u));
-          }
-          uint4* dh_ = reinterpret_cast<uint4*>(yp + co);
-          uint4* dl_ = reinterpret_cast<uint4*>(yp + p.Cout + co);
-          dh_[0] = make_uint4(hw[0], hw[1], hw[2], hw[3]); dh_[1] = make_uint4(hw[4], hw[5], hw[6], hw[7]);
-          dl_[0] = make_uint4(lw[0], lw[1], lw[2], lw[3]); dl_[1] = make_uint4(lw[4], lw[5], lw[6], lw[7]);
+        } else {
+#pragma unroll
+          for (int e = 0; e < 16; ++e)
+            if (co + e < p.Cout) o[e] += __ldg(p.bias + co + e);
         }
       }
+      if (p.relu) {
+#pragma unroll
+        for (int e = 0; e < 16; ++e) o[e] = fmaxf(o[e], 0.f);
+      }
+      uint32_t hw[8], lw[8];
+#pragma unroll
+      for (int e = 0; e < 8; ++e) {
+        hw[e] = pack_bf16x2(o[2 * e], o[2 * e + 1]);
+        lw[e] = pack_bf16x2(o[2 * e] - __uint_as_float(hw[e] << 16), o[2 * e + 1] - __uint_as_float(hw[e] & 0xffff0000u));
+      }
+      uint4* dh_ = reinterpret_cast<uint4*>(yp + co);
+      uint4* dl_ = reinterpret_cast<uint4*>(yp + p.Cout + co);
+      dh_[0] = make_uint4(hw[0], hw[1], hw[2], hw[3]); dh_[1] = make_uint4(hw[4], hw[5], hw[6], hw[7]);
+      dl_[0] = make_uint4(lw[0], lw[1], lw[2], lw[3]); dl_[1] = make_uint4(lw[4], lw[5], lw[6], lw[7]);
     }
   }
 }
diff --git a/upsnet_b200/csrc/tc_ptx.cuh b/upsnet_b200/csrc/tc_ptx.cuh
--- a/upsnet_b200/csrc/tc_ptx.cuh
+++ b/upsnet_b200/csrc/tc_ptx.cuh
@@ -115,6 +115,26 @@
         "wgmma.mma_async.sync.aligned.m64n256k16.f32.bf16.bf16 {%0, %1, %2, %3, %4, %5, %6, %7, %8, %9, %10, %11, %12, %13, %14, %15, %16, %17, %18, %19, %20, %21, %22, %23, %24, %25, %26, %27, %28, %29, %30, %31, %32, %33, %34, %35, %36, %37, %38, %39, %40, %41, %42, %43, %44, %45, %46, %47, %48, %49, %50, %51, %52, %53, %54, %55, %56, %57, %58, %59, %60, %61, %62, %63, %64, %65, %66, %67, %68, %69, %70, %71, %72, %73, %74, %75, %76, %77, %78, %79, %80, %81, %82, %83, %84, %85, %86, %87, %88, %89, %90, %91, %92, %93, %94, %95, %96, %97, %98, %99, %100, %101, %102, %103, %104, %105, %106, %107, %108, %109, %110, %111, %112, %113, %114, %115, %116, %117, %118, %119, %120, %121, %122, %123, %124, %125, %126, %127}, %128, %129, p, 1, 1, 0, 0;\n\t}"
         : "+f"(d[0]), "+f"(d[1]), "+f"(d[2]), "+f"(d[3]), "+f"(d[4]), "+f"(d[5]), "+f"(d[6]), "+f"(d[7]), "+f"(d[8]), "+f"(d[9]), "+f"(d[10]), "+f"(d[11]), "+f"(d[12]), "+f"(d[13]), "+f"(d[14]), "+f"(d[15]), "+f"(d[16]), "+f"(d[17]), "+f"(d[18]), "+f"(d[19]), "+f"(d[20]), "+f"(d[21]), "+f"(d[22]), "+f"(d[23]), "+f"(d[24]), "+f"(d[25]), "+f"(d[26]), "+f"(d[27]), "+f"(d[28]), "+f"(d[29]), "+f"(d[30]), "+f"(d[31]), "+f"(d[32]), "+f"(d[33]), "+f"(d[34]), "+f"(d[35]), "+f"(d[36]), "+f"(d[37]), "+f"(d[38]), "+f"(d[39]), "+f"(d[40]), "+f"(d[41]), "+f"(d[42]), "+f"(d[43]), "+f"(d[44]), "+f"(d[45]), "+f"(d[46]), "+f"(d[47]), "+f"(d[48]), "+f"(d[49]), "+f"(d[50]), "+f"(d[51]), "+f"(d[52]), "+f"(d[53]), "+f"(d[54]), "+f"(d[55]), "+f"(d[56]), "+f"(d[57]), "+f"(d[58]), "+f"(d[59]), "+f"(d[60]), "+f"(d[61]), "+f"(d[62]), "+f"(d[63]), "+f"(d[64]), "+f"(d[65]), "+f"(d[66]), "+f"(d[67]), "+f"(d[68]), "+f"(d[69]), "+f"(d[70]), "+f"(d[71]), "+f"(d[72]), "+f"(d[73]), "+f"(d[74]), "+f"(d[75]), "+f"(d[76]), "+f"(d[77]), "+f"(d[78]), "+f"(d[79]), "+f"(d[80]), "+f"(d[81]), "+f"(d[82]), "+f"(d[83]), "+f"(d[84]), "+f"(d[85]), "+f"(d[86]), "+f"(d[87]), "+f"(d[88]), "+f"(d[89]), "+f"(d[90]), "+f"(d[91]), "+f"(d[92]), "+f"(d[93]), "+f"(d[94]), "+f"(d[95]), "+f"(d[96]), "+f"(d[97]), "+f"(d[98]), "+f"(d[99]), "+f"(d[100]), "+f"(d[101]), "+f"(d[102]), "+f"(d[103]), "+f"(d[104]), "+f"(d[105]), "+f"(d[106]), "+f"(d[107]), "+f"(d[108]), "+f"(d[109]), "+f"(d[110]), "+f"(d[111]), "+f"(d[112]), "+f"(d[113]), "+f"(d[114]), "+f"(d[115]), "+f"(d[116]), "+f"(d[117]), "+f"(d[118]), "+f"(d[119]), "+f"(d[120]), "+f"(d[121]), "+f"(d[122]), "+f"(d[123]), "+f"(d[124]), "+f"(d[125]), "+f"(d[126]), "+f"(d[127])
         : "l"(da), "l"(db), "r"(accumulate));
+  }
+};
+
+template <int N> struct WgmmaRS;
+template <> struct WgmmaRS<32> {
+  static __device__ __forceinline__ void mma(float (&d)[16], const uint32_t (&a)[4], uint64_t db, uint32_t accumulate) {
+    asm volatile(
+        "{\n\t.reg .pred p;\n\tsetp.ne.b32 p, %21, 0;\n\t"
+        "wgmma.mma_async.sync.aligned.m64n32k16.f32.bf16.bf16 {%0, %1, %2, %3, %4, %5, %6, %7, %8, %9, %10, %11, %12, %13, %14, %15}, {%16, %17, %18, %19}, %20, p, 1, 1, 0;\n\t}"
+        : "+f"(d[0]), "+f"(d[1]), "+f"(d[2]), "+f"(d[3]), "+f"(d[4]), "+f"(d[5]), "+f"(d[6]), "+f"(d[7]), "+f"(d[8]), "+f"(d[9]), "+f"(d[10]), "+f"(d[11]), "+f"(d[12]), "+f"(d[13]), "+f"(d[14]), "+f"(d[15])
+        : "r"(a[0]), "r"(a[1]), "r"(a[2]), "r"(a[3]), "l"(db), "r"(accumulate));
+  }
+};
+template <> struct WgmmaRS<128> {
+  static __device__ __forceinline__ void mma(float (&d)[64], const uint32_t (&a)[4], uint64_t db, uint32_t accumulate) {
+    asm volatile(
+        "{\n\t.reg .pred p;\n\tsetp.ne.b32 p, %69, 0;\n\t"
+        "wgmma.mma_async.sync.aligned.m64n128k16.f32.bf16.bf16 {%0, %1, %2, %3, %4, %5, %6, %7, %8, %9, %10, %11, %12, %13, %14, %15, %16, %17, %18, %19, %20, %21, %22, %23, %24, %25, %26, %27, %28, %29, %30, %31, %32, %33, %34, %35, %36, %37, %38, %39, %40, %41, %42, %43, %44, %45, %46, %47, %48, %49, %50, %51, %52, %53, %54, %55, %56, %57, %58, %59, %60, %61, %62, %63}, {%64, %65, %66, %67}, %68, p, 1, 1, 0;\n\t}"
+        : "+f"(d[0]), "+f"(d[1]), "+f"(d[2]), "+f"(d[3]), "+f"(d[4]), "+f"(d[5]), "+f"(d[6]), "+f"(d[7]), "+f"(d[8]), "+f"(d[9]), "+f"(d[10]), "+f"(d[11]), "+f"(d[12]), "+f"(d[13]), "+f"(d[14]), "+f"(d[15]), "+f"(d[16]), "+f"(d[17]), "+f"(d[18]), "+f"(d[19]), "+f"(d[20]), "+f"(d[21]), "+f"(d[22]), "+f"(d[23]), "+f"(d[24]), "+f"(d[25]), "+f"(d[26]), "+f"(d[27]), "+f"(d[28]), "+f"(d[29]), "+f"(d[30]), "+f"(d[31]), "+f"(d[32]), "+f"(d[33]), "+f"(d[34]), "+f"(d[35]), "+f"(d[36]), "+f"(d[37]), "+f"(d[38]), "+f"(d[39]), "+f"(d[40]), "+f"(d[41]), "+f"(d[42]), "+f"(d[43]), "+f"(d[44]), "+f"(d[45]), "+f"(d[46]), "+f"(d[47]), "+f"(d[48]), "+f"(d[49]), "+f"(d[50]), "+f"(d[51]), "+f"(d[52]), "+f"(d[53]), "+f"(d[54]), "+f"(d[55]), "+f"(d[56]), "+f"(d[57]), "+f"(d[58]), "+f"(d[59]), "+f"(d[60]), "+f"(d[61]), "+f"(d[62]), "+f"(d[63])
+        : "r"(a[0]), "r"(a[1]), "r"(a[2]), "r"(a[3]), "l"(db), "r"(accumulate));
   }
 };
 
@@ -156,6 +176,10 @@
   asm volatile("ld.shared.v4.u32 {%0, %1, %2, %3}, [%4];" : "=r"(v.x), "=r"(v.y), "=r"(v.z), "=r"(v.w) : "r"(addr));
   return v;
 }
+__device__ __forceinline__ void ldsm_x4(uint32_t addr, uint32_t (&r)[4]) {
+  asm volatile("ldmatrix.sync.aligned.m8n8.x4.shared.b16 {%0, %1, %2, %3}, [%4];"
+               : "=r"(r[0]), "=r"(r[1]), "=r"(r[2]), "=r"(r[3]) : "r"(addr));
+}
 __device__ __forceinline__ void sts128(uint32_t addr, const uint4& v) {
   asm volatile("st.shared.v4.u32 [%0], {%1, %2, %3, %4};" ::"r"(addr), "r"(v.x), "r"(v.y), "r"(v.z), "r"(v.w) : "memory");
 }
```
